# kcat/openal-soft

Measured on NVIDIA H100. Metric: voice-samples/s mixed (HRTF, bsinc24, 1024-frame updates), higher is better.
Workload: dtype f32

## Files before the change

### openal-soft_b200/csrc/b200mix.cu

```cuda
#include "../../include/b200mix.h"

#include <algorithm>
#include <cmath>
#include <cstdio>
#include <cstdlib>
#include <cstring>
#include <new>
#include <string>
#include <vector>

#include <cuda_runtime.h>

#include <dlfcn.h>

#include "mixer_kernels.cuh"
#include "effect_kernels.cuh"
#include "shard_kernels.cuh"
#include "panmix_tc.cuh"
#include "param_kernels.hpp"
#include "efx_kernels.hpp"
#include "resampler_tables.hpp"
#include "hrtf_store.hpp"
#include "adpcm.hpp"

using namespace b200mix;

namespace {

thread_local std::string g_create_error;

struct DevBuf {
    void *ptr{nullptr}; size_t bytes{0};
};

}

struct b200mix_device {
    b200mix_device_desc desc{};
    int cuda_dev{0};
    int num_sms{0};
    cudaStream_t stream{nullptr};
    std::string error;
    uint64_t launches{0};

    BsincTable bsinc[3];
    float *d_bsinc[3]{};
    float *d_cubic[2]{};

    VoiceRec *d_voices{nullptr};
    BufferRec *d_buffers{nullptr};
    std::vector<BufferRec> h_buffers;
    std::vector<uint32_t> h_vbuf;
    std::vector<uint32_t> h_bufrefs;
    float2 *d_hrtf_tgt{nullptr}, *d_hrtf_old{nullptr};
    float *d_dry_cur{nullptr}, *d_dry_tgt{nullptr}, *d_send_cur{nullptr}, *d_send_tgt{nullptr};
    VoiceResult *d_results{nullptr};
    b200mix_voice_result *h_results{nullptr};
    char *d_outblock{nullptr}, *h_outblock{nullptr}; size_t out_real_bytes{0};

    uint32_t dry_alloc_ch{0};
    float *d_dry{nullptr}, *d_real{nullptr}, *d_wet{nullptr};
    float *d_partial{nullptr}; size_t partial_floats{0};
    float *d_accum_sum{nullptr};
    float *d_carry[2]{};
    int carry_idx{0};
    float *h_real{nullptr};

    uint32_t dec_channels{0}, dec_ir{0};
    float2 *d_dec_coef{nullptr}; float *d_dec_hfscale{nullptr}, *d_dec_state{nullptr};
    float *d_temp{nullptr}, *d_temp2{nullptr};
    uint32_t amb_in{0}; bool amb_dual{false};
    float *d_amb_hf{nullptr}, *d_amb_lf{nullptr}, *d_amb_state{nullptr};
    bool dry_active{false};
    float *d_uhj_state{nullptr}, *d_uhj_scratch{nullptr};
    uint32_t stab_center{B200MIX_NO_SLOT};
    float stab_coeff{0.0f};
    float *d_stab_state{nullptr};
    uint32_t bs2b_level{0};
    float *d_bs2b{nullptr};
    uint32_t uhj_fir{0};
    float *d_uhj_fir_state{nullptr}, *d_uhj_fir_coef{nullptr};

    char *h_arena{nullptr}, *d_arena{nullptr};
    VoiceUpdate *h_upd{nullptr};
    uint32_t stage_cap{0};
    cudaEvent_t stage_done{nullptr};
    bool stage_busy{false};

    std::vector<SlotRec> h_slots;
    SlotRec *d_slots{nullptr};
    std::vector<std::vector<void*>> slot_allocs;
    uint32_t active_slots{0};
    float *d_xscratch{nullptr};
    uint32_t *d_sendinfo{nullptr};
    FilterRec *d_filt{nullptr};
    FilterUpdate *h_fupd{nullptr}, *d_fupd{nullptr};
    uint32_t fupd_cap{0};
    cudaEvent_t fstage_done{nullptr};
    bool fstage_busy{false};
    float *d_fscratch{nullptr};
    uint32_t fscratch_rows{0};
    float *d_dline{nullptr};
    std::vector<uint8_t> h_dfilt;
    std::vector<uint32_t> h_order2;
    uint32_t *d_order2{nullptr};
    uint32_t num_order2{0};
    bool order2_dirty{false};
    std::vector<uint32_t> h_send_slot;
    std::vector<uint32_t> h_slot_start;
    std::vector<SendEntry> h_entries;
    uint32_t *d_slot_start{nullptr};
    SendEntry *d_entries{nullptr};
    uint32_t num_entries{0};
    bool sends_dirty{true};
    struct EfxHost { bool used{false}; EfxParams p{}; EfxDev *dev{nullptr}; uint32_t mod_index{0}, mod_range{1};
        uint32_t lfo_offset{0}, lfo_range{1}; };
    std::vector<EfxHost> efx;
    EfxSlotView *d_efx_views{nullptr};
    uint32_t efx_slots{0};
    uint32_t pshift_slots{0};
    bool efx_ready{false};
    float2 *d_twiddle{nullptr};
    float *d_cubic_filter{nullptr};
    uint32_t reverb_slots{0};

    float2 *d_st_fields{nullptr}; uint2 *d_st_elevs{nullptr}; float2 *d_st_coeffs{nullptr};
    uint8_t *d_st_delays{nullptr}; uint32_t st_num_fields{0}, st_ir{0};
    uint4 *d_qhdr{nullptr}; uint32_t *d_queue{nullptr};
    LimiterDev *d_limiter{nullptr};
    float *d_limiter_delay{nullptr};
    uint32_t *d_dc_delay{nullptr}; float *d_dc_gain{nullptr}, *d_dc_buf{nullptr};
    void *d_outbuf{nullptr}, *h_outbuf{nullptr};
    struct RvHost {
        bool used{false};
        int cur{0}, state{4};
        uint32_t fade[2]{1u, 1u};
        uint32_t offset{0};
        ReverbDev h[2];
        ReverbDev *dev{nullptr};
    };
    std::vector<RvHost> rv;
    std::vector<uint32_t> h_target;
    uint32_t num_stages{1}; bool any_target{false};
    bool reverb_upmix{false};
    bool mid_render{false}; uint32_t mid_frames{0};
    bool real_overwrite{false};
    std::vector<uint8_t> h_hrtf;
    std::vector<SendEntry> h_dry_entries;
    SendEntry *d_dry_entries{nullptr};
    uint32_t *d_dry_slot_start{nullptr};
    uint32_t num_dry_entries{0};
    bool dry_entries_dirty{true};
    float *d_dry_partial{nullptr};
    float *d_dry_geff{nullptr};
    float *d_send_geff{nullptr};
    float4 *d_dry_gramp{nullptr}, *d_send_gramp{nullptr};
    float *d_send_partial{nullptr};
    uint32_t send_partial_chunks{0}, max_slot_entries{0};
    bool profile{false};
    cudaEvent_t ev_mix0{nullptr}, ev_mix1{nullptr};
    bool ev_valid{false};
    static constexpr int kStages = 8;
    cudaEvent_t ev_stage[kStages + 1]{};
    bool stage_valid{false}; int profile_level{0};

    std::vector<uint8_t> h_active;
    std::vector<uint32_t> h_cost;
    std::vector<uint32_t> h_order;
    uint32_t *d_order{nullptr};
    uint32_t num_order{0};
    bool order_dirty{true};

    char *h_src{nullptr}, *d_src{nullptr}; uint32_t src_cap{0};
    cudaEvent_t src_done{nullptr}; bool src_busy{false};
    bool dev_filters{false};
    bool panmix_tc{false};
    bool mix_gather_only{false};

    struct Shard {
        uint32_t rank{0}, world{1}; int transport{0};
        char *own{nullptr}; size_t bytes{0};
        char *peer[kShardMaxWorld]{};
        size_t off_real{0}, off_wet{0}, real_floats{0}, wet_src_floats{0};
        uint32_t owned_max{0};
        uint32_t epoch{0};
        uint32_t *d_counters{nullptr};
        uint32_t *h_status{nullptr};
        cudaEvent_t ev[4]{};
        bool ev_wet{false}, ev_real{false};
        void *nccl_lib{nullptr}; void *comm{nullptr};
        int (*reduce)(const void*, void*, size_t, int, int, int, void*, cudaStream_t){nullptr};
        int (*allreduce)(const void*, void*, size_t, int, int, void*, cudaStream_t){nullptr};
        int (*comm_destroy)(void*){nullptr};
    } shard;

    uint32_t ir_pad{0};
    uint32_t voice_hi{0};
    int mix_variant{0}; int mix_groups{2}; int mix_gs{64}; int mix_cdr{0};
    uint32_t reverb_seq{0};
    size_t mix_smem{0}; int mix_blocks_per_sm{1};
};

namespace {

#define CUDA_TRY(dev, expr) do { cudaError_t e_ = (expr); if(e_ != cudaSuccess) {            \
    (dev)->error = std::string(#expr) + ": " + cudaGetErrorString(e_); return B200MIX_ERR_CUDA; } } while(0)

template<typename T>
int dev_alloc(b200mix_device *d, T *&p, size_t count, bool zero = true)
{
    p = nullptr;
    if(count == 0) return B200MIX_OK;
    CUDA_TRY(d, cudaMalloc(reinterpret_cast<void**>(&p), count*sizeof(T)));
    if(zero) CUDA_TRY(d, cudaMemsetAsync(p, 0, count*sizeof(T), d->stream));
    return B200MIX_OK;
}

using MixKernel = void(*)(const MixParams);

struct Variant { MixKernel fn; int gs, groups, cdr; size_t smem; bool hrtf; };

template<int GS, int GROUPS, bool HRTF, int CDR, int OPT, int FP>
Variant make_variant()
{
    return Variant{k_mix_voices<GS, GROUPS, HRTF, CDR, OPT, FP>, GS, GROUPS, CDR,
        sizeof(GroupSmem<GS, OPT, FP>)*GROUPS, HRTF};
}

Variant get_variant(int idx)
{
    switch(idx)
    {
    case 0: return make_variant<64, 2, true, 0, 17, 64>();
    case 1: return make_variant<64, 2, true, 0, 19, 128>();
    case 2: return make_variant<64, 2, false, 4, 1, 8>();
    default: return make_variant<64, 2, false, 0, 1, 8>();
    }
}

constexpr uint32_t kDryChunksMax = 128;

int ensure_dry_park(b200mix_device *d)
{
    const b200mix_device_desc &dd = d->desc;
    if(d->d_dry_entries) return B200MIX_OK;
    if(!d->d_xscratch)
        if(int rc = dev_alloc(d, d->d_xscratch, size_t(dd.max_voices)*kLine)) return rc;
    if(!d->d_sendinfo)
        if(int rc = dev_alloc(d, d->d_sendinfo, dd.max_voices)) return rc;
    if(int rc = dev_alloc(d, d->d_dry_entries, dd.max_voices)) return rc;
    if(dd.dry_channels > 4u && dd.dry_channels <= uint32_t(kPmN))
    {
        CUDA_TRY(d, cudaFuncSetAttribute(k_panmix_tc, cudaFuncAttributeMaxDynamicSharedMemorySize,
            kPmStages*kPmStageBytes + 1024));
        const char *simt = std::getenv("B200MIX_PANMIX_SIMT");
        d->panmix_tc = !(simt && simt[0] == '1');
    }
    if(int rc = dev_alloc(d, d->d_dry_slot_start, 2)) return rc;
    if(int rc = dev_alloc(d, d->d_dry_partial, size_t(kDryChunksMax)*dd.dry_channels*kLine)) return rc;
    if(int rc = dev_alloc(d, d->d_dry_geff, size_t(dd.max_voices)*dd.dry_channels)) return rc;
    if(int rc = dev_alloc(d, d->d_dry_gramp, size_t(dd.max_voices)*dd.dry_channels)) return rc;
    return B200MIX_OK;
}

static size_t align16(size_t v) { return (v + 15u) & ~size_t(15); }

int ensure_stage(b200mix_device *d, uint32_t n)
{
    if(n <= d->stage_cap) return B200MIX_OK;
    const b200mix_device_desc &dd = d->desc;
    if(d->stage_cap)
    {
        cudaStreamSynchronize(d->stream);
        cudaFreeHost(d->h_arena); cudaFree(d->d_arena);
        d->h_arena = nullptr; d->d_arena = nullptr;
    }
    const uint32_t cap = std::max<uint32_t>(n, 256u);
    const size_t bytes = align16(size_t(cap)*sizeof(VoiceUpdate))
        + align16(size_t(cap)*std::max<size_t>(size_t(dd.ir_size)*2, 4)*sizeof(float))
        + align16(size_t(cap)*dd.dry_channels*sizeof(float))
        + align16(size_t(cap)*dd.num_sends*dd.wet_channels*sizeof(float)) + 64;
    CUDA_TRY(d, cudaMallocHost(reinterpret_cast<void**>(&d->h_arena), bytes));
    CUDA_TRY(d, cudaMalloc(reinterpret_cast<void**>(&d->d_arena), bytes));
    d->h_upd = reinterpret_cast<VoiceUpdate*>(d->h_arena);
    d->stage_cap = cap;
    return B200MIX_OK;
}

const BsincTable *bsinc_for(const b200mix_device *d, uint32_t resampler)
{
    if(resampler < B200MIX_RESAMPLER_FAST_BSINC12 || resampler > B200MIX_RESAMPLER_BSINC48)
        return nullptr;
    return &d->bsinc[(resampler - B200MIX_RESAMPLER_FAST_BSINC12) >> 1];
}

}

extern "C" {

static void shard_release(b200mix_device *d);
static int ensure_filters(b200mix_device *d);

uint32_t b200mix_version(void) { return (1u<<16) | 1u; }

const char *b200mix_last_error(const b200mix_device *dev)
{ return dev ? dev->error.c_str() : g_create_error.c_str(); }

int b200mix_create(const b200mix_device_desc *desc, b200mix_device **out)
{
    if(!desc || !out || desc->struct_size != sizeof(b200mix_device_desc))
    { g_create_error = "bad descriptor"; return B200MIX_ERR_INVALID; }
    if(desc->dry_channels > B200MIX_MAX_DRY_CHANNELS || desc->wet_channels > B200MIX_MAX_WET_CHANNELS
        || desc->num_sends > B200MIX_MAX_SENDS || desc->ir_size > B200MIX_HRIR_LENGTH
        || desc->real_channels > B200MIX_MAX_DRY_CHANNELS || desc->max_voices == 0)
    { g_create_error = "descriptor out of range"; return B200MIX_ERR_INVALID; }
    if((desc->post_process == B200MIX_POST_UHJ && desc->dry_channels < 3)
        || (desc->post_process == B200MIX_POST_TSME && desc->dry_channels < 4))
    { g_create_error = "UHJ post-process needs W,X,Y dry channels"; return B200MIX_ERR_INVALID; }
    if((desc->post_process == B200MIX_POST_HRTF || desc->post_process == B200MIX_POST_UHJ
        || desc->post_process == B200MIX_POST_TSME)
        && (desc->real_left >= desc->real_channels || desc->real_right >= desc->real_channels))
    { g_create_error = "real_left/real_right outside RealOut"; return B200MIX_ERR_INVALID; }

    auto *d = new(std::nothrow) b200mix_device{};
    if(!d) { g_create_error = "out of host memory"; return B200MIX_ERR_NOMEM; }
    d->desc = *desc;
    if(const char *g = std::getenv("B200MIX_MIX_GATHER")) d->mix_gather_only = g[0] == '1';
    auto fail = [&](int code) { g_create_error = d->error; b200mix_destroy(d); return code; };

    int count = 0;
    if(cudaGetDeviceCount(&count) != cudaSuccess || count < 1)
    { d->error = "no CUDA device: the b200mix mixer has no CPU path"; return fail(B200MIX_ERR_CUDA); }
    if(desc->cuda_device >= 0) d->cuda_dev = desc->cuda_device;
    else if(cudaGetDevice(&d->cuda_dev) != cudaSuccess) d->cuda_dev = 0;
    if(cudaSetDevice(d->cuda_dev) != cudaSuccess)
    { d->error = "cudaSetDevice failed"; return fail(B200MIX_ERR_CUDA); }
    cudaDeviceProp prop{};
    if(cudaGetDeviceProperties(&prop, d->cuda_dev) != cudaSuccess)
    { d->error = "cudaGetDeviceProperties failed"; return fail(B200MIX_ERR_CUDA); }
    d->num_sms = prop.multiProcessorCount;
    if(cudaStreamCreateWithFlags(&d->stream, cudaStreamNonBlocking) != cudaSuccess)
    { d->error = "cudaStreamCreate failed"; return fail(B200MIX_ERR_CUDA); }
    if(cudaEventCreateWithFlags(&d->stage_done, cudaEventDisableTiming) != cudaSuccess)
    { d->error = "cudaEventCreate failed"; return fail(B200MIX_ERR_CUDA); }

    auto run = [&]() -> int {
        d->bsinc[0] = BuildBsincTable(60, 11, 2);
        d->bsinc[1] = BuildBsincTable(60, 23, 2);
        d->bsinc[2] = BuildBsincTable(80, 47, 1);
        for(int i = 0;i < 3;++i)
        {
            if(int rc = dev_alloc(d, d->d_bsinc[i], d->bsinc[i].tab.size(), false)) return rc;
            CUDA_TRY(d, cudaMemcpyAsync(d->d_bsinc[i], d->bsinc[i].tab.data(),
                d->bsinc[i].tab.size()*sizeof(float), cudaMemcpyHostToDevice, d->stream));
        }
        const std::vector<float> cubic[2] = {BuildSplineTable(), BuildGaussianTable()};
        for(int i = 0;i < 2;++i)
        {
            if(int rc = dev_alloc(d, d->d_cubic[i], cubic[i].size(), false)) return rc;
            CUDA_TRY(d, cudaMemcpyAsync(d->d_cubic[i], cubic[i].data(), cubic[i].size()*sizeof(float),
                cudaMemcpyHostToDevice, d->stream));
        }
        CUDA_TRY(d, cudaStreamSynchronize(d->stream));

        const b200mix_device_desc &dd = d->desc;
        d->ir_pad = (dd.ir_size + 7u) & ~7u;
        if(int rc = dev_alloc(d, d->d_voices, dd.max_voices)) return rc;
        if(int rc = dev_alloc(d, d->d_buffers, std::max(dd.max_buffers, 1u))) return rc;
        d->h_buffers.assign(std::max(dd.max_buffers, 1u), BufferRec{});
        d->h_vbuf.assign(dd.max_voices, B200MIX_NO_SLOT);
        d->h_bufrefs.assign(std::max(dd.max_buffers, 1u), 0u);
        if(dd.ir_size)
        {
            if(int rc = dev_alloc(d, d->d_hrtf_tgt, size_t(dd.max_voices)*d->ir_pad)) return rc;
            if(int rc = dev_alloc(d, d->d_hrtf_old, size_t(dd.max_voices)*d->ir_pad)) return rc;
        }
        if(int rc = dev_alloc(d, d->d_dry_cur, size_t(dd.max_voices)*std::max(dd.dry_channels, 1u))) return rc;
        if(int rc = dev_alloc(d, d->d_dry_tgt, size_t(dd.max_voices)*std::max(dd.dry_channels, 1u))) return rc;
        if(dd.num_sends && dd.wet_channels)
        {
            const size_t per = size_t(dd.num_sends)*dd.wet_channels;
            if(int rc = dev_alloc(d, d->d_send_cur, dd.max_voices*per)) return rc;
            if(int rc = dev_alloc(d, d->d_send_tgt, dd.max_voices*per)) return rc;
        }
        if(int rc = dev_alloc(d, d->d_order, dd.max_voices)) return rc;
        d->h_active.assign(dd.max_voices, 0);
        d->h_cost.assign(dd.max_voices, 0);
        d->h_hrtf.assign(dd.max_voices, 0);

        const bool hrtfDev = dd.ir_size > 0;
        d->mix_variant = hrtfDev ? (dd.ir_size <= 64 ? 0 : 1) : (dd.dry_channels <= 4 ? 2 : 3);
        const Variant var = get_variant(d->mix_variant);
        d->mix_gs = var.gs; d->mix_groups = var.groups; d->mix_cdr = var.cdr; d->mix_smem = var.smem;
        CUDA_TRY(d, cudaFuncSetAttribute(var.fn, cudaFuncAttributeMaxDynamicSharedMemorySize, int(var.smem)));
        int perSm = 0;
        CUDA_TRY(d, cudaOccupancyMaxActiveBlocksPerMultiprocessor(&perSm, var.fn, var.gs*var.groups, var.smem));
        d->mix_blocks_per_sm = std::max(perSm, 1);

        d->dry_alloc_ch = std::max<uint32_t>(std::max(dd.dry_channels, 1u), uint32_t(var.cdr));
        if(int rc = dev_alloc(d, d->d_dry, size_t(d->dry_alloc_ch)*kLine)) return rc;
        {
            const size_t realFloats = size_t(std::max(dd.real_channels, 1u))*kLine;
            static_assert(sizeof(VoiceResult) == 16 && sizeof(b200mix_voice_result) == 16, "result layout");
            const size_t blockBytes = realFloats*sizeof(float) + size_t(dd.max_voices)*sizeof(VoiceResult);
            char *blk = nullptr;
            if(int rc = dev_alloc(d, blk, blockBytes)) return rc;
            d->d_outblock = blk;
            d->d_results = reinterpret_cast<VoiceResult*>(blk + realFloats*sizeof(float));
            CUDA_TRY(d, cudaMallocHost(reinterpret_cast<void**>(&d->h_outblock), blockBytes));
            d->h_real = reinterpret_cast<float*>(d->h_outblock);
            d->h_results = reinterpret_cast<b200mix_voice_result*>(d->h_outblock + realFloats*sizeof(float));
            d->out_real_bytes = realFloats*sizeof(float);
            if(dd.post_process == B200MIX_POST_NONE) d->d_real = d->d_dry;
            else d->d_real = reinterpret_cast<float*>(blk);
        }
        if(dd.max_slots && dd.wet_channels)
            if(int rc = dev_alloc(d, d->d_wet, size_t(dd.max_slots)*dd.wet_channels*kLine)) return rc;
        const size_t maxRows = size_t(d->num_sms)*d->mix_blocks_per_sm;
        d->partial_floats = maxRows*(hrtfDev ? 2*kAccumLen : 0) + maxRows*size_t(var.cdr)*kLine;
        if(int rc = dev_alloc(d, d->d_partial, std::max<size_t>(2*d->partial_floats, 4))) return rc;
        if(int rc = dev_alloc(d, d->d_accum_sum, 2*kAccumLen)) return rc;
        if(int rc = dev_alloc(d, d->d_carry[0], 2*kHrirLen)) return rc;
        if(int rc = dev_alloc(d, d->d_carry[1], 2*kHrirLen)) return rc;
        if(int rc = dev_alloc(d, d->d_temp, size_t(std::max(dd.dry_channels, 1u))*kLine)) return rc;
        if(int rc = dev_alloc(d, d->d_temp2, size_t(std::max(dd.dry_channels, 1u))*kLine)) return rc;
        if(dd.max_slots && dd.wet_channels && dd.num_sends)
        {
            d->h_slots.assign(dd.max_slots, SlotRec{});
            d->slot_allocs.assign(dd.max_slots, {});
            if(int rc = dev_alloc(d, d->d_slots, dd.max_slots)) return rc;
            if(int rc = dev_alloc(d, d->d_xscratch, size_t(dd.max_voices)*kLine)) return rc;
            if(int rc = dev_alloc(d, d->d_sendinfo, dd.max_voices)) return rc;
            if(int rc = dev_alloc(d, d->d_send_geff, size_t(dd.max_voices)*dd.num_sends*dd.wet_channels)) return rc;
            if(int rc = dev_alloc(d, d->d_send_gramp, size_t(dd.max_voices)*dd.num_sends*dd.wet_channels)) return rc;
            d->h_send_slot.assign(size_t(dd.max_voices)*B200MIX_MAX_SENDS, B200MIX_NO_SLOT);
            if(int rc = dev_alloc(d, d->d_slot_start, dd.max_slots + 1)) return rc;
            if(int rc = dev_alloc(d, d->d_entries, size_t(dd.max_voices)*dd.num_sends)) return rc;
            std::vector<float2> tw(128);
            for(int k = 0;k < 128;++k)
            {
                const double a = -2.0*3.14159265358979323846*double(k)/256.0;
                tw[k] = make_float2(float(std::cos(a)), float(std::sin(a)));
            }
            const std::vector<float> cf = BuildCubicFilter();
            if(int rc = dev_alloc(d, d->d_cubic_filter, cf.size(), false)) return rc;
            CUDA_TRY(d, cudaMemcpyAsync(d->d_cubic_filter, cf.data(), cf.size()*sizeof(float),
                cudaMemcpyHostToDevice, d->stream));
            CUDA_TRY(d, cudaStreamSynchronize(d->stream));
            if(int rc = dev_alloc(d, d->d_twiddle, 128, false)) return rc;
            CUDA_TRY(d, cudaMemcpyAsync(d->d_twiddle, tw.data(), 128*sizeof(float2),
                cudaMemcpyHostToDevice, d->stream));
            CUDA_TRY(d, cudaStreamSynchronize(d->stream));
        }
        if(dd.post_process == B200MIX_POST_UHJ || dd.post_process == B200MIX_POST_TSME)
        {
            if(int rc = dev_alloc(d, d->d_uhj_state, 64)) return rc;
            if(int rc = dev_alloc(d, d->d_uhj_scratch, 5*1025)) return rc;
        }
        if(int rc = ensure_stage(d, std::min(dd.max_voices, 4096u))) return rc;
        CUDA_TRY(d, cudaStreamSynchronize(d->stream));
        return B200MIX_OK;
    };
    int rc;
    try { rc = run(); }
    catch(const std::exception &e) { d->error = e.what(); rc = B200MIX_ERR_NOMEM; }
    if(rc != B200MIX_OK) return fail(rc);
    *out = d;
    return B200MIX_OK;
}

void b200mix_destroy(b200mix_device *d)
{
    if(!d) return;
    if(d->stream) cudaStreamSynchronize(d->stream);
    shard_release(d);
    for(auto &b : d->h_buffers) if(b.data) cudaFree(const_cast<void*>(b.data));
    for(int i = 0;i < 3;++i) cudaFree(d->d_bsinc[i]);
    for(int i = 0;i < 2;++i) cudaFree(d->d_cubic[i]);
    cudaFree(d->d_voices); cudaFree(d->d_buffers); cudaFree(d->d_hrtf_tgt); cudaFree(d->d_hrtf_old);
    cudaFree(d->d_dry_cur); cudaFree(d->d_dry_tgt); cudaFree(d->d_send_cur); cudaFree(d->d_send_tgt);
    cudaFree(d->d_outblock); cudaFreeHost(d->h_outblock); cudaFree(d->d_order);
    cudaFree(d->d_dry); cudaFree(d->d_wet); cudaFree(d->d_partial); cudaFree(d->d_accum_sum);
    cudaFree(d->d_carry[0]); cudaFree(d->d_carry[1]);
    cudaFree(d->d_dec_coef); cudaFree(d->d_dec_hfscale); cudaFree(d->d_dec_state);
    cudaFree(d->d_temp); cudaFree(d->d_temp2);
    cudaFree(d->d_amb_hf); cudaFree(d->d_amb_lf); cudaFree(d->d_amb_state);
    cudaFree(d->d_uhj_state); cudaFree(d->d_uhj_scratch);
    cudaFree(d->d_uhj_fir_state); cudaFree(d->d_uhj_fir_coef); cudaFree(d->d_bs2b); cudaFree(d->d_stab_state);
    for(auto &v : d->slot_allocs) for(void *p : v) cudaFree(p);
    cudaFree(d->d_slots); cudaFree(d->d_xscratch); cudaFree(d->d_sendinfo);
    cudaFree(d->d_filt); cudaFree(d->d_fupd); cudaFree(d->d_fscratch);
    cudaFree(d->d_dline); cudaFree(d->d_order2); cudaFree(d->d_qhdr); cudaFree(d->d_queue);
    cudaFree(d->d_outbuf); if(d->h_outbuf) cudaFreeHost(d->h_outbuf);
    cudaFree(d->d_limiter); cudaFree(d->d_limiter_delay);
    cudaFree(d->d_dc_delay); cudaFree(d->d_dc_gain); cudaFree(d->d_dc_buf);
    cudaFree(d->d_st_fields); cudaFree(d->d_st_elevs); cudaFree(d->d_st_coeffs); cudaFree(d->d_st_delays);
    cudaFree(d->d_dry_entries); cudaFree(d->d_dry_slot_start); cudaFree(d->d_dry_partial);
    cudaFree(d->d_dry_geff); cudaFree(d->d_send_geff); cudaFree(d->d_send_partial);
    cudaFree(d->d_dry_gramp); cudaFree(d->d_send_gramp);
    if(d->h_fupd) cudaFreeHost(d->h_fupd);
    if(d->fstage_done) cudaEventDestroy(d->fstage_done);
    cudaFree(d->d_slot_start); cudaFree(d->d_entries); cudaFree(d->d_twiddle); cudaFree(d->d_cubic_filter);
    cudaFree(d->d_efx_views);
    cudaFreeHost(d->h_arena); cudaFree(d->d_arena);
    if(d->h_src) cudaFreeHost(d->h_src);
    cudaFree(d->d_src);
    if(d->src_done) cudaEventDestroy(d->src_done);
    if(d->stage_done) cudaEventDestroy(d->stage_done);
    if(d->ev_mix0) cudaEventDestroy(d->ev_mix0);
    if(d->ev_mix1) cudaEventDestroy(d->ev_mix1);
    for(cudaEvent_t e : d->ev_stage) if(e) cudaEventDestroy(e);
    if(d->stream) cudaStreamDestroy(d->stream);
    delete d;
}

int b200mix_set_hrtf_decoder(b200mix_device *d, uint32_t channels, uint32_t ir_size,
    const float *coeffs, const float *hf_scale, const float *splitter_coeff)
{
    if(!d || channels != d->desc.dry_channels || ir_size > B200MIX_HRIR_LENGTH || !coeffs
        || !hf_scale || !splitter_coeff || d->desc.post_process != B200MIX_POST_HRTF)
    { if(d) d->error = "set_hrtf_decoder: bad arguments"; return B200MIX_ERR_INVALID; }
    CUDA_TRY(d, cudaSetDevice(d->cuda_dev));
    cudaFree(d->d_dec_coef); cudaFree(d->d_dec_hfscale); cudaFree(d->d_dec_state);
    d->dec_channels = channels; d->dec_ir = ir_size;
    if(int rc = dev_alloc(d, d->d_dec_coef, size_t(channels)*ir_size, false)) return rc;
    if(int rc = dev_alloc(d, d->d_dec_hfscale, channels, false)) return rc;
    if(int rc = dev_alloc(d, d->d_dec_state, size_t(channels)*4)) return rc;
    std::vector<float> st(size_t(channels)*4, 0.0f);
    for(uint32_t c = 0;c < channels;++c) st[c*4] = splitter_coeff[c];
    CUDA_TRY(d, cudaMemcpyAsync(d->d_dec_coef, coeffs, size_t(channels)*ir_size*2*sizeof(float),
        cudaMemcpyHostToDevice, d->stream));
    CUDA_TRY(d, cudaMemcpyAsync(d->d_dec_hfscale, hf_scale, channels*sizeof(float),
        cudaMemcpyHostToDevice, d->stream));
    CUDA_TRY(d, cudaMemcpyAsync(d->d_dec_state, st.data(), st.size()*sizeof(float),
        cudaMemcpyHostToDevice, d->stream));
    CUDA_TRY(d, cudaStreamSynchronize(d->stream));
    return B200MIX_OK;
}

int b200mix_set_ambi_decoder(b200mix_device *d, uint32_t in_channels, const float *gains_hf,
    const float *gains_lf, float xover_coeff)
{
    if(!d || in_channels != d->desc.dry_channels || !gains_hf
        || d->desc.post_process != B200MIX_POST_AMBIDEC)
    { if(d) d->error = "set_ambi_decoder: bad arguments"; return B200MIX_ERR_INVALID; }
    CUDA_TRY(d, cudaSetDevice(d->cuda_dev));
    cudaFree(d->d_amb_hf); cudaFree(d->d_amb_lf); cudaFree(d->d_amb_state);
    d->d_amb_lf = nullptr;
    const size_t n = size_t(in_channels)*d->desc.real_channels;
    d->amb_in = in_channels; d->amb_dual = gains_lf != nullptr;
    if(int rc = dev_alloc(d, d->d_amb_hf, n, false)) return rc;
    CUDA_TRY(d, cudaMemcpyAsync(d->d_amb_hf, gains_hf, n*sizeof(float), cudaMemcpyHostToDevice, d->stream));
    if(gains_lf)
    {
        if(int rc = dev_alloc(d, d->d_amb_lf, n, false)) return rc;
        CUDA_TRY(d, cudaMemcpyAsync(d->d_amb_lf, gains_lf, n*sizeof(float), cudaMemcpyHostToDevice, d->stream));
    }
    std::vector<float> st(size_t(in_channels)*4, 0.0f);
    for(uint32_t c = 0;c < in_channels;++c) st[c*4] = xover_coeff;
    if(int rc = dev_alloc(d, d->d_amb_state, st.size(), false)) return rc;
    CUDA_TRY(d, cudaMemcpyAsync(d->d_amb_state, st.data(), st.size()*sizeof(float),
        cudaMemcpyHostToDevice, d->stream));
    CUDA_TRY(d, cudaStreamSynchronize(d->stream));
    return B200MIX_OK;
}

int b200mix_buffer_data(b200mix_device *d, uint32_t buffer, uint32_t sample_type, uint32_t channels,
    uint32_t frames, const void *data, size_t bytes)
{
    if(!d) return B200MIX_ERR_INVALID;
    static const size_t sz[] = {1, 2, 4, 4, 8, 1, 1};
    if(buffer >= d->desc.max_buffers || sample_type > B200MIX_FMT_ALAW || channels < 1 || !data)
    { d->error = "buffer_data: bad arguments"; return B200MIX_ERR_INVALID; }
    const size_t need = size_t(frames)*channels*sz[sample_type];
    if(bytes < need) { d->error = "buffer_data: short data"; return B200MIX_ERR_INVALID; }
    CUDA_TRY(d, cudaSetDevice(d->cuda_dev));
    BufferRec &h = d->h_buffers[buffer];
    if(h.data && d->h_bufrefs[buffer])
    { d->error = "buffer_data: the buffer is attached to an active voice (AL_INVALID_OPERATION)"; return B200MIX_ERR_INVALID; }
    if(h.data)
    {
        CUDA_TRY(d, cudaStreamSynchronize(d->stream));
        cudaFree(const_cast<void*>(h.data));
        h = BufferRec{};
    }
    void *p = nullptr;
    CUDA_TRY(d, cudaMalloc(&p, need + 16));
    CUDA_TRY(d, cudaMemcpyAsync(p, data, need, cudaMemcpyHostToDevice, d->stream));
    h.data = p; h.frames = frames; h.type = sample_type; h.channels = channels;
    CUDA_TRY(d, cudaMemcpyAsync(d->d_buffers + buffer, &h, sizeof(BufferRec), cudaMemcpyHostToDevice,
        d->stream));
    return B200MIX_OK;
}

int b200mix_buffer_data_adpcm(b200mix_device *d, uint32_t buffer, uint32_t sample_type,
    uint32_t channels, uint32_t samples_per_block, uint32_t blocks, const void *data, size_t bytes)
{
    if(!d) return B200MIX_ERR_INVALID;
    const bool ms = sample_type == B200MIX_FMT_MSADPCM;
    if((sample_type != B200MIX_FMT_IMA4 && !ms) || channels < 1 || channels > 2 || !data
        || !AdpcmBlockValid(ms, samples_per_block))
    { d->error = "buffer_data_adpcm: bad arguments"; return B200MIX_ERR_INVALID; }
    if(bytes < AdpcmBlockBytes(ms, channels, samples_per_block)*blocks
        || uint64_t(blocks)*samples_per_block > 0x7fffffffull)
    { d->error = "buffer_data_adpcm: short data"; return B200MIX_ERR_INVALID; }
    std::vector<int16_t> pcm(size_t(blocks)*samples_per_block*channels);
    if(ms) DecodeMSADPCM(static_cast<const uint8_t*>(data), channels, samples_per_block, blocks, pcm.data());
    else DecodeIMA4(static_cast<const uint8_t*>(data), channels, samples_per_block, blocks, pcm.data());
    const int rc = b200mix_buffer_data(d, buffer, B200MIX_FMT_I16, channels, blocks*samples_per_block,
        pcm.data(), pcm.size()*sizeof(int16_t));
    if(rc == B200MIX_OK) CUDA_TRY(d, cudaStreamSynchronize(d->stream));
    return rc;
}

int b200mix_buffer_free(b200mix_device *d, uint32_t buffer)
{
    if(!d || buffer >= d->desc.max_buffers) return B200MIX_ERR_INVALID;
    CUDA_TRY(d, cudaSetDevice(d->cuda_dev));
    BufferRec &h = d->h_buffers[buffer];
    if(h.data && d->h_bufrefs[buffer])
    { d->error = "buffer_free: the buffer is attached to an active voice; stop the voice first"; return B200MIX_ERR_INVALID; }
    if(h.data)
    {
        CUDA_TRY(d, cudaStreamSynchronize(d->stream));
        cudaFree(const_cast<void*>(h.data));
        h = BufferRec{};
        CUDA_TRY(d, cudaMemcpyAsync(d->d_buffers + buffer, &h, sizeof(BufferRec),
            cudaMemcpyHostToDevice, d->stream));
    }
    return B200MIX_OK;
}

static int update_stages(b200mix_device *d)
{
    const uint32_t ns = uint32_t(d->h_slots.size());
    if(d->h_target.size() != ns) d->h_target.assign(ns, B200MIX_NO_SLOT);
    std::vector<uint32_t> depth(ns, 0);
    uint32_t maxd = 0; d->any_target = false;
    for(uint32_t sl = 0;sl < ns;++sl)
    {
        uint32_t hops = 0;
        for(uint32_t t = d->h_target[sl];t != B200MIX_NO_SLOT && hops <= ns;t = d->h_target[t]) ++hops;
        depth[sl] = hops;
        if(d->h_slots[sl].type) { maxd = std::max(maxd, hops); if(hops) d->any_target = true; }
    }
    d->num_stages = maxd + 1u;
    for(uint32_t sl = 0;sl < ns;++sl)
    {
        d->h_slots[sl].stage = d->h_slots[sl].type ? maxd - std::min(depth[sl], maxd) : 0u;
        d->h_slots[sl].target = d->h_target[sl];
    }
    if(ns && d->d_slots)
    {
        CUDA_TRY(d, cudaMemcpyAsync(d->d_slots, d->h_slots.data(), ns*sizeof(SlotRec), cudaMemcpyHostToDevice, d->stream));
        CUDA_TRY(d, cudaStreamSynchronize(d->stream));
    }
    if(ns && d->d_efx_views)
    {
        std::vector<EfxSlotView> views(ns, EfxSlotView{nullptr, nullptr, 0u, 0u});
        for(uint32_t sl = 0;sl < ns;++sl)
            if(d->h_slots[sl].type >= B200MIX_EFFECT_ECHO && sl < d->efx.size() && d->efx[sl].used)
                views[sl] = EfxSlotView{d->efx[sl].dev, d->h_slots[sl].lines, d->h_slots[sl].stage, 0u};
        CUDA_TRY(d, cudaMemcpyAsync(d->d_efx_views, views.data(), ns*sizeof(EfxSlotView), cudaMemcpyHostToDevice, d->stream));
        CUDA_TRY(d, cudaStreamSynchronize(d->stream));
    }
    return B200MIX_OK;
}

static void free_slot(b200mix_device *d, uint32_t slot)
{
    cudaStreamSynchronize(d->stream);
    for(void *p : d->slot_allocs[slot]) cudaFree(p);
    d->slot_allocs[slot].clear();
    if(d->h_slots[slot].type) --d->active_slots;
    if(d->h_slots[slot].type == B200MIX_EFFECT_REVERB) --d->reverb_slots;
    if(d->h_slots[slot].type >= B200MIX_EFFECT_ECHO)
    {
        --d->efx_slots;
        if(d->h_slots[slot].type == B200MIX_EFFECT_PSHIFTER) --d->pshift_slots;
        if(slot < d->efx.size()) d->efx[slot] = b200mix_device::EfxHost{};
    }
    if(slot < d->rv.size()) d->rv[slot].used = false;
    d->h_slots[slot] = SlotRec{};
    if(d->d_slots)
    {
        cudaMemcpyAsync(d->d_slots + slot, &d->h_slots[slot], sizeof(SlotRec), cudaMemcpyHostToDevice, d->stream);
        cudaStreamSynchronize(d->stream);
    }
}

int b200mix_slot_disable(b200mix_device *d, uint32_t slot)
{
    if(!d || slot >= d->h_slots.size()) { if(d) d->error = "slot_disable: bad slot"; return B200MIX_ERR_INVALID; }
    CUDA_TRY(d, cudaSetDevice(d->cuda_dev));
    free_slot(d, slot);
    return update_stages(d);
}

int b200mix_slot_convolution(b200mix_device *d, uint32_t slot, uint32_t ir_channels,
    uint32_t ir_frames, const float *ir)
{
    if(!d || slot >= d->h_slots.size() || !ir_channels || ir_channels > 16 || !ir_frames || !ir)
    { if(d) d->error = "slot_convolution: bad arguments (or the device has no sends/slots)"; return B200MIX_ERR_INVALID; }
    CUDA_TRY(d, cudaSetDevice(d->cuda_dev));
    free_slot(d, slot);
    CUDA_TRY(d, cudaFuncSetAttribute(k_conv_mac, cudaFuncAttributeMaxDynamicSharedMemorySize, int(sizeof(ConvMacSmem))));
    SlotRec r{};
    r.type = B200MIX_EFFECT_CONVOLUTION; r.channels = ir_channels; r.frames = ir_frames;
    const uint32_t nseg = std::max<uint32_t>((ir_frames + kConvBlock - 1)/kConvBlock, 2u) - 1u;
    r.segs = nseg;
    auto alloc = [&](auto *&p, size_t count) -> int {
        if(int rc = dev_alloc(d, p, count)) return rc;
        d->slot_allocs[slot].push_back(p);
        return B200MIX_OK;
    };
    if(int rc = alloc(r.H, size_t(ir_channels)*nseg*kConvFft)) return rc;
    if(int rc = alloc(r.X, size_t(nseg + kConvMaxBlocks)*kConvFft)) return rc;
    if(int rc = alloc(r.head, size_t(ir_channels)*kConvBlock)) return rc;
    if(int rc = alloc(r.inbuf, kConvFft)) return rc;
    if(int rc = alloc(r.ov, size_t(ir_channels)*kConvFft)) return rc;
    if(int rc = alloc(r.yspec, size_t(ir_channels)*kConvMaxChunks*kConvMaxBlocks*kConvFft)) return rc;
    if(int rc = alloc(r.lines, size_t(ir_channels)*kLine)) return rc;
    if(int rc = alloc(r.gains, size_t(2)*ir_channels*32)) return rc;
    if(int rc = alloc(r.gtgt, size_t(ir_channels)*32)) return rc;

    std::vector<float> H(size_t(ir_channels)*nseg*kConvFft, 0.0f), head(size_t(ir_channels)*kConvBlock, 0.0f);
    std::vector<double> cs(kConvFft), sn(kConvFft);
    for(int k = 0;k < kConvFft;++k)
    {
        cs[k] = std::cos(2.0*3.14159265358979323846*k/kConvFft);
        sn[k] = std::sin(2.0*3.14159265358979323846*k/kConvFft);
    }
    for(uint32_t c = 0;c < ir_channels;++c)
    {
        const float *h = ir + size_t(c)*ir_frames;
        for(uint32_t k = 0;k < uint32_t(kConvBlock) && k < ir_frames;++k) head[c*kConvBlock + k] = h[k];
        for(uint32_t sg = 0;sg < nseg;++sg)
        {
            const size_t base = size_t(kConvBlock)*(sg + 1);
            float *dst = H.data() + (size_t(c)*nseg + sg)*kConvFft;
            const uint32_t cnt = base < ir_frames ? std::min<uint32_t>(kConvBlock, uint32_t(ir_frames - base)) : 0u;
            for(int bin = 0;bin <= kConvBlock;++bin)
            {
                double re = 0.0, im = 0.0;
                for(uint32_t j = 0;j < cnt;++j)
                {
                    const int ph = int((uint64_t(bin)*j) % kConvFft);
                    re += double(h[base + j])*cs[ph];
                    im -= double(h[base + j])*sn[ph];
                }
                const double sc = 1.0/double(kConvFft);
                if(bin == 0) dst[0] = float(re*sc);
                else if(bin == kConvBlock) dst[1] = float(re*sc);
                else { dst[bin*2] = float(re*sc); dst[bin*2+1] = float(im*sc); }
            }
        }
    }
    CUDA_TRY(d, cudaMemcpyAsync(r.H, H.data(), H.size()*sizeof(float), cudaMemcpyHostToDevice, d->stream));
    CUDA_TRY(d, cudaMemcpyAsync(r.head, head.data(), head.size()*sizeof(float), cudaMemcpyHostToDevice, d->stream));
    d->h_slots[slot] = r;
    CUDA_TRY(d, cudaMemcpyAsync(d->d_slots + slot, &d->h_slots[slot], sizeof(SlotRec), cudaMemcpyHostToDevice, d->stream));
    CUDA_TRY(d, cudaStreamSynchronize(d->stream));
    ++d->active_slots;
    d->dry_active = true;
    return update_stages(d);
}

static void reverb_fill_params(ReverbDev &h, const b200mix_reverb_params *p)
{
    std::memcpy(h.early_tap, p->early_tap, sizeof(h.early_tap)); h.early_tap_coeff = p->early_tap_coeff;
    std::memcpy(h.late_tap, p->late_tap, sizeof(h.late_tap));
    h.mix_x = p->mix_x; h.mix_y = p->mix_y;
    std::memcpy(h.filter_lp, p->filter_lp, sizeof(h.filter_lp));
    std::memcpy(h.filter_hp, p->filter_hp, sizeof(h.filter_hp));
    h.early_ap_coeff = p->early_ap_coeff;
    std::memcpy(h.early_ap_offset, p->early_ap_offset, sizeof(h.early_ap_offset));
    std::memcpy(h.early_offset, p->early_offset, sizeof(h.early_offset));
    h.early_coeff = p->early_coeff;
    std::memcpy(h.late_offset, p->late_offset, sizeof(h.late_offset));
    h.density_gain = p->density_gain;
    std::memcpy(h.t60_mid_gain, p->t60_mid_gain, sizeof(h.t60_mid_gain));
    std::memcpy(h.t60_hf, p->t60_hf, sizeof(h.t60_hf)); std::memcpy(h.t60_lf, p->t60_lf, sizeof(h.t60_lf));
    h.mod_step = p->mod_step; h.mod_depth = p->mod_depth; h.late_ap_coeff = p->late_ap_coeff;
    std::memcpy(h.late_ap_offset, p->late_ap_offset, sizeof(h.late_ap_offset));
    h.upmix = p->upmix ? 1u : 0u; h.order_scale[0] = p->order_scale[0]; h.order_scale[1] = p->order_scale[1];
    h.split_coeff = p->splitter_coeff;
}

static int reverb_check_params(b200mix_device *d, const b200mix_reverb_params *p)
{
    auto pow2 = [](uint32_t v) { return v >= 4u && !(v & (v-1u)); };
    if(!pow2(p->main_len) || !pow2(p->late_in_len) || !pow2(p->early_ap_len) || !pow2(p->early_len)
        || !pow2(p->late_ap_len) || !pow2(p->late_len) || !p->late_offset[0] || !p->late_ap_offset[0])
// ... 551 lines not shown
                if(int rc = ensure_dry_park(d)) return rc;
        }
        const uint8_t hv = hrtfMode ? 1 : 0;
        if(d->h_hrtf[p.voice] != hv) { d->h_hrtf[p.voice] = hv; d->dry_entries_dirty = true; }
        const uint8_t act = stopped ? 0 : 1;
        uint32_t cost = p.resampler >= 2u ? 4u : 2u;
        if(const BsincTable *t = bsinc_for(d, p.resampler)) cost = t->m[0];
        if(d->h_active[p.voice] != act || (!d->h_cost[p.voice] && act)) { d->order_dirty = true; d->h_cost[p.voice] = cost; }
        d->h_active[p.voice] = act;
        d->voice_hi = std::max(d->voice_hi, p.voice + 1u);
        const uint32_t nb = (!stopped && (p.flags & B200MIX_VF_STATIC)) ? p.buffer : B200MIX_NO_SLOT;
        uint32_t &ob = d->h_vbuf[p.voice];
        if(ob != nb)
        {
            if(ob != B200MIX_NO_SLOT) --d->h_bufrefs[ob];
            if(nb != B200MIX_NO_SLOT) ++d->h_bufrefs[nb];
            ob = nb;
        }
    }

    const uint32_t paths = 1u + dd.num_sends;
    const size_t inBytes = align16(size_t(n)*sizeof(b200mix_source_voice)) + align16(size_t(n)*sizeof(b200mix_source_props));
    if(d->src_busy) { CUDA_TRY(d, cudaEventSynchronize(d->src_done)); d->src_busy = false; }
    if(n > d->src_cap)
    {
        CUDA_TRY(d, cudaStreamSynchronize(d->stream));
        if(d->h_src) cudaFreeHost(d->h_src);
        cudaFree(d->d_src); d->h_src = nullptr; d->d_src = nullptr;
        const uint32_t cap = std::max(n, 2u*d->src_cap);
        const size_t in = align16(size_t(cap)*sizeof(b200mix_source_voice)) + align16(size_t(cap)*sizeof(b200mix_source_props));
        const size_t out = align16(size_t(cap)*sizeof(VoiceUpdate)) + align16(size_t(cap)*16)
            + align16(size_t(cap)*std::max(dd.dry_channels, 1u)*4) + align16(size_t(cap)*std::max(dd.num_sends*dd.wet_channels, 1u)*4)
            + align16(size_t(cap)*(1u + B200MIX_MAX_SENDS)*8) + align16(size_t(cap)*paths*sizeof(FilterUpdate));
        CUDA_TRY(d, cudaMallocHost(reinterpret_cast<void**>(&d->h_src), in));
        CUDA_TRY(d, cudaMalloc(reinterpret_cast<void**>(&d->d_src), in + out + 64));
        if(!d->src_done) CUDA_TRY(d, cudaEventCreateWithFlags(&d->src_done, cudaEventDisableTiming));
        d->src_cap = cap;
    }
    std::memcpy(d->h_src, voices, size_t(n)*sizeof(b200mix_source_voice));
    const size_t offProps = align16(size_t(n)*sizeof(b200mix_source_voice));
    std::memcpy(d->h_src + offProps, props, size_t(n)*sizeof(b200mix_source_props));
    CUDA_TRY(d, cudaMemcpyAsync(d->d_src, d->h_src, inBytes, cudaMemcpyHostToDevice, d->stream));
    CUDA_TRY(d, cudaEventRecord(d->src_done, d->stream));
    d->src_busy = true;

    CalcVoicesParams Q{};
    Q.voices = reinterpret_cast<const b200mix_source_voice*>(d->d_src);
    Q.props = reinterpret_cast<const b200mix_source_props*>(d->d_src + offProps);
    Q.n = n; Q.listener = *listener;
    Q.device_rate = env->device_rate; Q.num_sends = dd.num_sends; Q.render_mode = env->render_mode;
    Q.cd = dd.dry_channels; Q.cw = dd.wet_channels; Q.ir = dd.ir_size;
    if(!hrtfMode)
    {
        Q.dry_channels = env->dry.channels;
        for(uint32_t c = 0;c < env->dry.channels;++c) { Q.dry_scale[c] = env->dry.scale[c]; Q.dry_index[c] = env->dry.index[c]; }
    }
    for(uint32_t s = 0;s < dd.num_sends;++s)
    {
        Q.wet_channels[s] = env->wet[s].channels;
        for(uint32_t c = 0;c < env->wet[s].channels;++c) { Q.wet_scale[s][c] = env->wet[s].scale[c]; Q.wet_index[s][c] = env->wet[s].index[c]; }
    }
    for(int t = 0;t < 3;++t)
    {
        Q.bsinc[t].scaleBase = d->bsinc[t].scaleBase; Q.bsinc[t].scaleRange = d->bsinc[t].scaleRange;
        for(unsigned k = 0;k < kBsincScales;++k) { Q.bsinc[t].m[k] = d->bsinc[t].m[k]; Q.bsinc[t].filterOffset[k] = d->bsinc[t].filterOffset[k]; }
    }
    size_t off = inBytes;
    auto carve = [&](size_t bytes) { char *p = d->d_src + off; off += align16(bytes); return p; };
    Q.updates = reinterpret_cast<VoiceUpdate*>(carve(size_t(n)*sizeof(VoiceUpdate)));
    Q.dirs = reinterpret_cast<float4*>(carve(size_t(n)*16));
    Q.dry = reinterpret_cast<float*>(carve(size_t(n)*std::max(dd.dry_channels, 1u)*4));
    Q.send = (dd.num_sends && dd.wet_channels)
        ? reinterpret_cast<float*>(carve(size_t(n)*dd.num_sends*dd.wet_channels*4)) : nullptr;
    Q.gains_hflf = reinterpret_cast<float*>(carve(size_t(n)*(1u + B200MIX_MAX_SENDS)*8));
    Q.fupd = reinterpret_cast<FilterUpdate*>(carve(size_t(n)*paths*sizeof(FilterUpdate)));
    const bool filters = d->d_filt != nullptr;
    CUDA_TRY(d, launch_calc_voices(Q, filters, d->stream));
    d->launches += filters ? 2 : 1;

    ApplyParams A{};
    A.voices = d->d_voices; A.updates = Q.updates;
    if(hrtfMode)
    {
        A.dirs = Q.dirs;
        A.st_fields = d->d_st_fields; A.st_elevs = d->d_st_elevs; A.st_coeffs = d->d_st_coeffs;
        A.st_delays = d->d_st_delays; A.st_num_fields = d->st_num_fields; A.st_ir = d->st_ir;
    }
    else A.dry = Q.dry;
    A.send = Q.send;
    A.hrtf_tgt = d->d_hrtf_tgt; A.hrtf_old = d->d_hrtf_old;
    A.dry_cur = d->d_dry_cur; A.dry_tgt = d->d_dry_tgt;
    A.send_cur = d->d_send_cur; A.send_tgt = d->d_send_tgt;
    A.ir = dd.ir_size; A.ir_pad = d->ir_pad; A.cd = dd.dry_channels; A.cw = dd.wet_channels;
    A.num_sends = dd.num_sends;
    A.filt = d->d_filt; A.filt_paths = paths;
    A.qhdr = d->d_qhdr;
    k_apply_updates<<<n, 64, 0, d->stream>>>(A);
    ++d->launches;
    if(filters)
    {
        k_apply_filter_updates<<<(2u*n*paths + 127u)/128u, 128, 0, d->stream>>>(d->d_filt, paths, Q.fupd, n*paths);
        ++d->launches;
    }
    CUDA_TRY(d, cudaGetLastError());
    return B200MIX_OK;
}

int b200mix_get_voice_targets(b200mix_device *d, uint32_t voice, uint32_t *step, float bsinc[4],
    float *hrtf_gain, uint32_t hrtf_delay[2], float *hrtf_coeffs, float *dry_gains, float *send_gains,
    float *filters)
{
    if(!d || voice >= d->desc.max_voices) return B200MIX_ERR_INVALID;
    const b200mix_device_desc &dd = d->desc;
    CUDA_TRY(d, cudaSetDevice(d->cuda_dev));
    CUDA_TRY(d, cudaStreamSynchronize(d->stream));
    VoiceRec rec;
    CUDA_TRY(d, cudaMemcpy(&rec, d->d_voices + voice, offsetof(VoiceRec, prev), cudaMemcpyDeviceToHost));
    if(step) *step = rec.step;
    if(bsinc)
    {
        bsinc[0] = rec.bsinc_sf;
        std::memcpy(&bsinc[1], &rec.bsinc_m, 4); std::memcpy(&bsinc[2], &rec.bsinc_l, 4);
        std::memcpy(&bsinc[3], &rec.bsinc_off, 4);
    }
    if(hrtf_gain) *hrtf_gain = rec.tgt_gain;
    if(hrtf_delay) { hrtf_delay[0] = rec.tgt_delay0; hrtf_delay[1] = rec.tgt_delay1; }
    if(hrtf_coeffs && d->d_hrtf_tgt)
        CUDA_TRY(d, cudaMemcpy(hrtf_coeffs, d->d_hrtf_tgt + size_t(voice)*d->ir_pad, size_t(dd.ir_size)*8, cudaMemcpyDeviceToHost));
    if(dry_gains && dd.dry_channels)
        CUDA_TRY(d, cudaMemcpy(dry_gains, d->d_dry_tgt + size_t(voice)*dd.dry_channels, size_t(dd.dry_channels)*4, cudaMemcpyDeviceToHost));
    if(send_gains && d->d_send_tgt)
        CUDA_TRY(d, cudaMemcpy(send_gains, d->d_send_tgt + size_t(voice)*dd.num_sends*dd.wet_channels,
            size_t(dd.num_sends)*dd.wet_channels*4, cudaMemcpyDeviceToHost));
    if(filters)
    {
        const uint32_t paths = 1u + dd.num_sends;
        for(uint32_t pth = 0;pth < paths;++pth)
        {
            float *o = filters + size_t(pth)*11;
            for(int k = 0;k < 11;++k) o[k] = k == 1 ? 1.0f : (k == 6 ? 1.0f : 0.0f);
            if(!d->d_filt) continue;
            FilterRec fr;
            CUDA_TRY(d, cudaMemcpy(&fr, d->d_filt + size_t(voice)*paths + pth, sizeof(fr), cudaMemcpyDeviceToHost));
            o[0] = fr.active ? 1.0f : 0.0f;
            for(int k = 0;k < 5;++k) { o[1+k] = fr.tgt[0][k]; o[6+k] = fr.tgt[1][k]; }
        }
    }
    return B200MIX_OK;
}

int b200mix_voice_queue(b200mix_device *d, uint32_t voice, uint32_t count, const uint32_t *buffers,
    uint32_t loop_index)
{
    if(!d) return B200MIX_ERR_INVALID;
    const b200mix_device_desc &dd = d->desc;
    if(voice >= dd.max_voices || (count && !buffers))
    { d->error = "voice_queue: bad arguments"; return B200MIX_ERR_INVALID; }
    if(count > B200MIX_MAX_QUEUE)
    { d->error = "voice_queue: more than B200MIX_MAX_QUEUE items"; return B200MIX_ERR_UNSUPPORTED; }
    if(loop_index != B200MIX_NO_LOOP && loop_index >= count)
    { d->error = "voice_queue: loop index outside the list"; return B200MIX_ERR_INVALID; }
    QueueSet Q{};
    Q.voice = voice; Q.count = count; Q.loop = loop_index;
    for(uint32_t i = 0;i < count;++i)
    {
        if(buffers[i] >= dd.max_buffers || !d->h_buffers[buffers[i]].data)
        { d->error = "voice_queue: buffer id without data"; return B200MIX_ERR_INVALID; }
        Q.items[i] = buffers[i];
    }
    CUDA_TRY(d, cudaSetDevice(d->cuda_dev));
    if(!d->d_qhdr)
    {
        if(int rc = dev_alloc(d, d->d_qhdr, dd.max_voices)) return rc;
        if(int rc = dev_alloc(d, d->d_queue, size_t(dd.max_voices)*kMaxQueue)) return rc;
    }
    k_set_queue<<<1, 32, 0, d->stream>>>(d->d_voices, d->d_qhdr, d->d_queue, Q);
    ++d->launches;
    CUDA_TRY(d, cudaGetLastError());
    return B200MIX_OK;
}

static int ensure_filters(b200mix_device *d)
{
    if(d->d_filt) return B200MIX_OK;
    const b200mix_device_desc &dd = d->desc;
    const uint32_t paths = 1u + dd.num_sends;
    const size_t count = size_t(dd.max_voices)*paths;
    if(int rc = dev_alloc(d, d->d_filt, count, false)) return rc;
    k_filter_init<<<unsigned((count*32u + 255u)/256u), 256, 0, d->stream>>>(d->d_filt, count);
    ++d->launches;
    CUDA_TRY(d, cudaGetLastError());
    CUDA_TRY(d, cudaEventCreateWithFlags(&d->fstage_done, cudaEventDisableTiming));
    if(!d->d_xscratch)
        if(int rc = dev_alloc(d, d->d_xscratch, size_t(dd.max_voices)*kLine)) return rc;
    if(!d->d_sendinfo)
        if(int rc = dev_alloc(d, d->d_sendinfo, dd.max_voices)) return rc;
    if(int rc = dev_alloc(d, d->d_dline, size_t(dd.max_voices)*kLine)) return rc;
    if(int rc = dev_alloc(d, d->d_order2, dd.max_voices)) return rc;
    d->h_dfilt.assign(dd.max_voices, 0);
    return B200MIX_OK;
}

int b200mix_voices_filters(b200mix_device *d, uint32_t n, const b200mix_voice_filter *filters)
{
    static_assert(sizeof(FilterUpdate) == sizeof(b200mix_voice_filter), "FilterUpdate mirrors the ABI struct");
    if(!d) return B200MIX_ERR_INVALID;
    if(n == 0) return B200MIX_OK;
    if(!filters) { d->error = "voices_filters: null filters"; return B200MIX_ERR_INVALID; }
    const b200mix_device_desc &dd = d->desc;
    const uint32_t paths = 1u + dd.num_sends;
    for(uint32_t i = 0;i < n;++i)
        if(filters[i].voice >= dd.max_voices || filters[i].path >= paths)
        { d->error = "voices_filters: voice/path out of range"; return B200MIX_ERR_INVALID; }
    CUDA_TRY(d, cudaSetDevice(d->cuda_dev));
    if(int rc = ensure_filters(d)) return rc;
    for(uint32_t i = 0;i < n;++i)
        if(filters[i].path == 0)
        {
            const uint8_t act = filters[i].active ? 1 : 0;
            if(d->h_dfilt[filters[i].voice] != act) { d->h_dfilt[filters[i].voice] = act; d->order2_dirty = true; }
        }
    if(d->fstage_busy)
    {
        CUDA_TRY(d, cudaEventSynchronize(d->fstage_done));
        d->fstage_busy = false;
    }
    if(n > d->fupd_cap)
    {
        CUDA_TRY(d, cudaStreamSynchronize(d->stream));
        if(d->h_fupd) cudaFreeHost(d->h_fupd);
        cudaFree(d->d_fupd);
        d->h_fupd = nullptr; d->d_fupd = nullptr;
        const uint32_t cap = std::max(n, 2u*d->fupd_cap);
        CUDA_TRY(d, cudaMallocHost(reinterpret_cast<void**>(&d->h_fupd), size_t(cap)*sizeof(FilterUpdate)));
        CUDA_TRY(d, cudaMalloc(reinterpret_cast<void**>(&d->d_fupd), size_t(cap)*sizeof(FilterUpdate)));
        d->fupd_cap = cap;
    }
    std::memcpy(d->h_fupd, filters, size_t(n)*sizeof(FilterUpdate));
    CUDA_TRY(d, cudaMemcpyAsync(d->d_fupd, d->h_fupd, size_t(n)*sizeof(FilterUpdate),
        cudaMemcpyHostToDevice, d->stream));
    k_apply_filter_updates<<<(2u*n + 127u)/128u, 128, 0, d->stream>>>(d->d_filt, paths, d->d_fupd, n);
    ++d->launches;
    CUDA_TRY(d, cudaGetLastError());
    CUDA_TRY(d, cudaEventRecord(d->fstage_done, d->stream));
    d->fstage_busy = true;
    return B200MIX_OK;
}

static inline void stage_mark(b200mix_device *d, int i)
{ if(d->profile_level >= 2) cudaEventRecord(d->ev_stage[i], d->stream); }

static int render_phase_a(b200mix_device *d, uint32_t frames, bool want_results, bool force_sends)
{
    const b200mix_device_desc &dd = d->desc;
    if(frames < 1 || frames > B200MIX_LINE_SIZE)
    { d->error = "render: frames out of range"; return B200MIX_ERR_INVALID; }
    if(dd.post_process == B200MIX_POST_HRTF && !d->dec_channels)
    { d->error = "render: HRTF decoder not set"; return B200MIX_ERR_INVALID; }
    if(dd.post_process == B200MIX_POST_AMBIDEC && !d->amb_in)
    { d->error = "render: ambisonic decoder not set"; return B200MIX_ERR_INVALID; }
    CUDA_TRY(d, cudaSetDevice(d->cuda_dev));

    stage_mark(d, 0);
    if(d->dry_active || dd.post_process != B200MIX_POST_HRTF)
        CUDA_TRY(d, cudaMemsetAsync(d->d_dry, 0, size_t(d->dry_alloc_ch)*kLine*sizeof(float), d->stream));
    d->real_overwrite = dd.post_process == B200MIX_POST_HRTF && dd.real_channels == 2
        && dd.real_left != dd.real_right;
    if(d->d_real != d->d_dry && !d->real_overwrite)
        CUDA_TRY(d, cudaMemsetAsync(d->d_real, 0, size_t(dd.real_channels)*kLine*sizeof(float), d->stream));
    if(d->d_wet)
        CUDA_TRY(d, cudaMemsetAsync(d->d_wet, 0, size_t(dd.max_slots)*dd.wet_channels*kLine*sizeof(float), d->stream));

    if(d->order_dirty)
    {
        d->h_order.clear();
        for(uint32_t v = 0;v < d->voice_hi;++v) if(d->h_active[v]) d->h_order.push_back(v);
        std::stable_sort(d->h_order.begin(), d->h_order.end(),
            [d](uint32_t a, uint32_t b) { return d->h_cost[a] > d->h_cost[b]; });
        d->num_order = uint32_t(d->h_order.size());
        if(d->num_order)
        {
            CUDA_TRY(d, cudaMemcpyAsync(d->d_order, d->h_order.data(), d->num_order*sizeof(uint32_t),
                cudaMemcpyHostToDevice, d->stream));
            CUDA_TRY(d, cudaStreamSynchronize(d->stream));
        }
        d->order_dirty = false;
        d->order2_dirty = true;
        d->dry_entries_dirty = true;
    }
    if(d->d_filt && d->order2_dirty)
    {
        d->h_order2.clear();
        for(uint32_t v : d->h_order) if(d->dev_filters || d->h_dfilt[v]) d->h_order2.push_back(v);
        d->num_order2 = uint32_t(d->h_order2.size());
        if(d->num_order2)
        {
            CUDA_TRY(d, cudaMemcpyAsync(d->d_order2, d->h_order2.data(), d->num_order2*sizeof(uint32_t),
                cudaMemcpyHostToDevice, d->stream));
            CUDA_TRY(d, cudaStreamSynchronize(d->stream));
        }
        d->order2_dirty = false;
    }
    const Variant var = get_variant(d->mix_variant);
    const uint32_t nv = std::max(d->voice_hi, 1u);
    const uint32_t maxBlocks = uint32_t(d->num_sms*d->mix_blocks_per_sm);
    const uint32_t blocks = std::max(1u, std::min(maxBlocks, (d->num_order + var.groups - 1)/var.groups));
    const size_t rows = size_t(blocks);

    MixParams P{};
    P.voices = d->d_voices; P.buffers = d->d_buffers;
    P.hrtf_tgt = d->d_hrtf_tgt; P.hrtf_old = d->d_hrtf_old;
    P.dry_cur = d->d_dry_cur; P.dry_tgt = d->d_dry_tgt;
    P.send_cur = d->d_send_cur; P.send_tgt = d->d_send_tgt;
    P.dry = d->d_dry; P.wet = d->d_wet; P.partial = d->d_partial;
    P.results = want_results ? d->d_results : nullptr;
    for(int i = 0;i < 3;++i) P.bsinc_tab[i] = d->d_bsinc[i];
    for(int i = 0;i < 2;++i) P.cubic_tab[i] = d->d_cubic[i];
    P.max_voices = nv; P.frames = frames; P.ir = dd.ir_size; P.ir_pad = d->ir_pad;
    P.cd = dd.dry_channels; P.cw = dd.wet_channels; P.num_sends = dd.num_sends;
    P.max_buffers = dd.max_buffers;
    P.order = d->d_order; P.num_order = d->num_order;
    P.xscratch = d->d_xscratch; P.sendinfo = d->d_sendinfo;
    P.filt = d->d_filt; P.filt_paths = 1u + dd.num_sends;
    P.qhdr = d->d_qhdr; P.queue = d->d_queue;
    P.gather_only = d->mix_gather_only ? 1u : 0u;
    stage_mark(d, 1);
    if(d->profile) cudaEventRecord(d->ev_mix0, d->stream);
    var.fn<<<blocks, var.gs*var.groups, var.smem, d->stream>>>(P);
    if(d->profile) { cudaEventRecord(d->ev_mix1, d->stream); d->ev_valid = true; }
    ++d->launches;
    CUDA_TRY(d, cudaGetLastError());

    stage_mark(d, 2);
    size_t rows2 = 0;
    if(d->d_filt && d->num_order2)
    {
        FilterRunParams FP{};
        FP.filt = d->d_filt; FP.filt_paths = 1u + dd.num_sends; FP.sendinfo = d->d_sendinfo;
        FP.direct_order = d->d_order2; FP.num_direct = d->num_order2;
        FP.xscratch = d->d_xscratch; FP.dline = d->d_dline; FP.frames = frames;
        k_filters<<<(d->num_order2 + 31u)/32u, 32, 0, d->stream>>>(FP);
        ++d->launches;
        const uint32_t blocks2 = std::max(1u, std::min(maxBlocks, (d->num_order2 + var.groups - 1)/var.groups));
        rows2 = blocks2;
        MixParams P2 = P;
        P2.pass = 1u; P2.dline = d->d_dline;
        P2.order = d->d_order2; P2.num_order = d->num_order2;
        P2.partial = d->d_partial + d->partial_floats;
        P2.results = nullptr;
        var.fn<<<blocks2, var.gs*var.groups, var.smem, d->stream>>>(P2);
        ++d->launches;
        CUDA_TRY(d, cudaGetLastError());
    }

    stage_mark(d, 3);
    if(var.hrtf)
    {
        const uint32_t len = 2*kAccumLen;
        k_reduce_rows<<<(len/4 + kReduceCols - 1)/kReduceCols, 1024, 0, d->stream>>>(d->d_partial, uint32_t(rows), len,
            d->d_accum_sum, 0);
        ++d->launches;
        if(rows2)
        {
            k_reduce_rows<<<(len/4 + kReduceCols - 1)/kReduceCols, 1024, 0, d->stream>>>(d->d_partial + d->partial_floats,
                uint32_t(rows2), len, d->d_accum_sum, 1);
            ++d->launches;
        }
    }
    if(var.cdr > 0)
    {
        const uint32_t len = uint32_t(var.cdr)*kLine;
        const float *pd = d->d_partial + (var.hrtf ? rows*(2*kAccumLen) : 0);
        k_reduce_rows<<<(len/4 + kReduceCols - 1)/kReduceCols, 1024, 0, d->stream>>>(pd, uint32_t(rows), len, d->d_dry, 1);
        ++d->launches;
        if(rows2)
        {
            const float *pd2 = d->d_partial + d->partial_floats + (var.hrtf ? rows2*(2*kAccumLen) : 0);
            k_reduce_rows<<<(len/4 + kReduceCols - 1)/kReduceCols, 1024, 0, d->stream>>>(pd2, uint32_t(rows2), len, d->d_dry, 1);
            ++d->launches;
        }
    }
    CUDA_TRY(d, cudaGetLastError());

    stage_mark(d, 4);
    if(var.cdr == 0 && d->d_dry_entries)
    {
        if(d->dry_entries_dirty)
        {
            d->h_dry_entries.clear();
            for(uint32_t v = 0;v < d->voice_hi;++v)
                if(d->h_active[v] && !d->h_hrtf[v]) d->h_dry_entries.push_back(SendEntry{v, 0u});
            d->num_dry_entries = uint32_t(d->h_dry_entries.size());
            const uint32_t ss[2] = {0u, d->num_dry_entries};
            CUDA_TRY(d, cudaMemcpyAsync(d->d_dry_slot_start, ss, sizeof(ss), cudaMemcpyHostToDevice, d->stream));
            if(d->num_dry_entries)
                CUDA_TRY(d, cudaMemcpyAsync(d->d_dry_entries, d->h_dry_entries.data(),
                    d->num_dry_entries*sizeof(SendEntry), cudaMemcpyHostToDevice, d->stream));
            CUDA_TRY(d, cudaStreamSynchronize(d->stream));
            d->dry_entries_dirty = false;
        }
        if(d->num_dry_entries)
        {
            SendMixParams DM{};
            DM.slot_start = d->d_dry_slot_start; DM.entries = d->d_dry_entries; DM.sendinfo = d->d_sendinfo;
            DM.xscratch = d->d_xscratch; DM.send_cur = d->d_dry_cur; DM.send_tgt = d->d_dry_tgt;
            DM.wet = d->d_dry; DM.frames = frames; DM.cw = dd.dry_channels; DM.num_sends = 1;
            DM.valid_bit = kSiDry; DM.dline = d->d_dline ? d->d_dline : d->d_xscratch;
            const uint32_t chunks = std::max(1u, std::min(kDryChunksMax, (d->num_dry_entries + 63u)/64u));
            DM.chunks = chunks; DM.partial = d->d_dry_partial; DM.geff = d->d_dry_geff; DM.gramp = d->d_dry_gramp;
            {
                const uint32_t tot = d->num_dry_entries*dd.dry_channels;
                k_send_gains_prepare<<<(tot + 127)/128, 128, 0, d->stream>>>(DM, d->num_dry_entries);
                ++d->launches;
            }
            const bool tc = d->panmix_tc && dd.dry_channels > 4u && dd.dry_channels <= uint32_t(kPmN)
                && frames == uint32_t(kLine) && chunks > 1u;
            const uint32_t tiles = tc ? 1u : (chunks > 1u ? uint32_t(kLine/128) : (frames + 127u)/128u);
            if(dd.dry_channels > 4u) k_send_mix<16><<<dim3(1, tiles, chunks), 256, 0, d->stream>>>(DM);
            else k_send_mix<4><<<dim3(1, tiles, chunks), 256, 0, d->stream>>>(DM);
            ++d->launches;
            if(tc)
            {
                PanMixTcParams TQ{d->d_dry_slot_start, d->d_dry_entries, d->d_sendinfo, d->d_xscratch,
                    d->d_dline, d->d_dry_geff, dd.dry_channels, chunks, d->d_dry_partial};
                k_panmix_tc<<<chunks, 128, kPmStages*kPmStageBytes + 1024, d->stream>>>(TQ);
                ++d->launches;
            }
            if(chunks > 1u)
            {
                const uint32_t len = dd.dry_channels*kLine;
                if(chunks <= 16u)
                    k_reduce_few<<<(len/4 + 255)/256, 256, 0, d->stream>>>(d->d_dry_partial, chunks, len, d->d_dry, 1);
                else
                k_reduce_rows<<<(len/4 + kReduceCols - 1)/kReduceCols, 1024, 0, d->stream>>>(
                    d->d_dry_partial, chunks, len, d->d_dry, 1);
                ++d->launches;
            }
            const uint32_t tot = d->num_dry_entries*dd.dry_channels;
            k_send_gains_update<<<(tot + 127)/128, 128, 0, d->stream>>>(DM, d->num_dry_entries);
            ++d->launches;
            CUDA_TRY(d, cudaGetLastError());
        }
    }

    stage_mark(d, 5);
    if((d->active_slots || force_sends) && d->d_wet && d->d_slot_start)
    {
        if(d->sends_dirty)
        {
            d->h_slot_start.assign(dd.max_slots + 1, 0);
            d->h_entries.clear();
            for(uint32_t sl = 0;sl < dd.max_slots;++sl)
            {
                d->h_slot_start[sl] = uint32_t(d->h_entries.size());
                for(uint32_t v = 0;v < d->voice_hi;++v)
                    for(uint32_t s2 = 0;s2 < dd.num_sends;++s2)
                        if(d->h_send_slot[size_t(v)*B200MIX_MAX_SENDS + s2] == sl)
                            d->h_entries.push_back(SendEntry{v, s2});
            }
            d->h_slot_start[dd.max_slots] = uint32_t(d->h_entries.size());
            d->num_entries = uint32_t(d->h_entries.size());
            d->max_slot_entries = 0;
            for(uint32_t sl = 0;sl < dd.max_slots;++sl)
                d->max_slot_entries = std::max(d->max_slot_entries, d->h_slot_start[sl+1] - d->h_slot_start[sl]);
            CUDA_TRY(d, cudaMemcpyAsync(d->d_slot_start, d->h_slot_start.data(),
                (dd.max_slots + 1)*sizeof(uint32_t), cudaMemcpyHostToDevice, d->stream));
            if(d->num_entries)
                CUDA_TRY(d, cudaMemcpyAsync(d->d_entries, d->h_entries.data(),
                    d->num_entries*sizeof(SendEntry), cudaMemcpyHostToDevice, d->stream));
            CUDA_TRY(d, cudaStreamSynchronize(d->stream));
            d->sends_dirty = false;
        }
        SendMixParams SM{};
        SM.slot_start = d->d_slot_start; SM.entries = d->d_entries; SM.sendinfo = d->d_sendinfo;
        SM.xscratch = d->d_xscratch; SM.send_cur = d->d_send_cur; SM.send_tgt = d->d_send_tgt;
        SM.wet = d->d_wet; SM.frames = frames; SM.cw = dd.wet_channels; SM.num_sends = dd.num_sends;
        SM.valid_bit = kSiSend; SM.chunks = 1;
        if(d->d_filt && d->num_entries)
        {
            if(d->fscratch_rows < d->num_entries)
            {
                CUDA_TRY(d, cudaStreamSynchronize(d->stream));
                cudaFree(d->d_fscratch); d->d_fscratch = nullptr; d->fscratch_rows = 0;
                const uint32_t rows = std::max(d->num_entries, 64u);
                CUDA_TRY(d, cudaMalloc(reinterpret_cast<void**>(&d->d_fscratch), size_t(rows)*kLine*sizeof(float)));
                CUDA_TRY(d, cudaMemsetAsync(d->d_fscratch, 0, size_t(rows)*kLine*sizeof(float), d->stream));
                d->fscratch_rows = rows;
            }
            SM.filt = d->d_filt; SM.filt_paths = 1u + dd.num_sends; SM.fscratch = d->d_fscratch;
            FilterRunParams FP{};
            FP.filt = d->d_filt; FP.filt_paths = 1u + dd.num_sends; FP.sendinfo = d->d_sendinfo;
            FP.entries = d->d_entries; FP.num_entries = d->num_entries;
            FP.xscratch = d->d_xscratch; FP.fscratch = d->d_fscratch; FP.frames = frames;
            k_filters<<<(d->num_entries + 31u)/32u, 32, 0, d->stream>>>(FP);
            ++d->launches;
        }
        SM.geff = d->d_send_geff; SM.gramp = d->d_send_gramp;
        if(d->num_entries)
        {
            const uint32_t tot = d->num_entries*dd.wet_channels;
            k_send_gains_prepare<<<(tot + 127)/128, 128, 0, d->stream>>>(SM, d->num_entries);
            ++d->launches;
        }
        {
            const uint32_t chunks = std::max(1u, std::min(16u, (d->max_slot_entries + 127u)/128u));
            if(chunks > 1u && d->send_partial_chunks < chunks)
            {
                CUDA_TRY(d, cudaStreamSynchronize(d->stream));
                cudaFree(d->d_send_partial); d->d_send_partial = nullptr; d->send_partial_chunks = 0;
                CUDA_TRY(d, cudaMalloc(reinterpret_cast<void**>(&d->d_send_partial),
                    size_t(chunks)*dd.max_slots*dd.wet_channels*kLine*sizeof(float)));
                d->send_partial_chunks = chunks;
            }
            SM.chunks = chunks; SM.partial = d->d_send_partial;
            const uint32_t tiles = chunks > 1u ? uint32_t(kLine/128) : (frames + 127u)/128u;
            if(dd.wet_channels > 4u) k_send_mix<16><<<dim3(dd.max_slots, tiles, chunks), 256, 0, d->stream>>>(SM);
            else k_send_mix<4><<<dim3(dd.max_slots, tiles, chunks), 256, 0, d->stream>>>(SM);
            ++d->launches;
            if(chunks > 1u)
            {
                const uint32_t len = dd.max_slots*dd.wet_channels*kLine;
                if(chunks <= 16u)
                    k_reduce_few<<<(len/4 + 255)/256, 256, 0, d->stream>>>(d->d_send_partial, chunks, len, d->d_wet, 1);
                else
                k_reduce_rows<<<(len/4 + kReduceCols - 1)/kReduceCols, 1024, 0, d->stream>>>(
                    d->d_send_partial, chunks, len, d->d_wet, 1);
                ++d->launches;
            }
        }
        if(d->num_entries)
        {
            const uint32_t tot = d->num_entries*dd.wet_channels;
            k_send_gains_update<<<(tot + 127)/128, 128, 0, d->stream>>>(SM, d->num_entries);
            ++d->launches;
        }
        CUDA_TRY(d, cudaGetLastError());
    }
    return B200MIX_OK;
}

static int render_phase_b(b200mix_device *d, uint32_t frames)
{
    const b200mix_device_desc &dd = d->desc;
    stage_mark(d, 6);
    if(d->active_slots)
    {
        ConvParams CP{};
        CP.slots = d->d_slots; CP.wet = d->d_wet; CP.twiddle = d->d_twiddle;
        CP.frames = frames; CP.cw = dd.wet_channels; CP.num_slots = dd.max_slots;
        uint32_t convCh = 1, convWork = 0, convSegs = 0;
        for(const SlotRec &sr : d->h_slots)
            if(sr.type == B200MIX_EFFECT_CONVOLUTION)
            { convCh = std::max(convCh, sr.channels); convWork += sr.channels; convSegs = std::max(convSegs, sr.segs); }
        CP.chunks = 1u;
        if(convWork)
            CP.chunks = std::max(1u, std::min(std::min(uint32_t(kConvMaxChunks), (convSegs + 17u)/18u),
                (4u*uint32_t(d->num_sms) + convWork - 1u)/convWork));
        if(d->reverb_slots)
        {
            for(uint32_t sl = 0;sl < d->rv.size();++sl)
            {
                b200mix_device::RvHost &R = d->rv[sl];
                if(!R.used || d->h_slots[sl].type != B200MIX_EFFECT_REVERB) continue;
                uint32_t mask = 1u << R.cur;
                if(R.state < 2) R.state = 2;
                if(R.state != 4)
                {
                    const int old = R.cur ^ 1;
                    if(R.state == 3)
                    {
                        if(int rc = reverb_clear_pipeline(d, sl, old)) return rc;
                        R.state = 4;
                    }
                    else
                    {
                        if(frames >= R.fade[old])
                        {
                            CUDA_TRY(d, cudaMemsetAsync(d->h_slots[sl].gtgt + size_t(old)*8*32, 0,
                                size_t(8)*32*sizeof(float), d->stream));
                            R.fade[old] = 0; R.state = 3;
                        }
                        else R.fade[old] -= frames;
                        mask |= 1u << old;
                    }
                }
                R.offset += frames;
                if(d->h_slots[sl].rv_mask != mask || d->h_slots[sl].rv_cur != uint32_t(R.cur))
                {
                    d->h_slots[sl].rv_mask = mask; d->h_slots[sl].rv_cur = uint32_t(R.cur);
                    CUDA_TRY(d, cudaMemcpyAsync(d->d_slots + sl, &d->h_slots[sl], sizeof(SlotRec),
                        cudaMemcpyHostToDevice, d->stream));
                    CUDA_TRY(d, cudaStreamSynchronize(d->stream));
                }
            }
        }
        SlotMixParams SP{};
        SP.slots = d->d_slots; SP.dry = d->d_dry; SP.frames = frames; SP.cd = dd.dry_channels;
        SP.num_slots = dd.max_slots; SP.wet = d->d_wet; SP.cw = dd.wet_channels;
        for(uint32_t st = 0;st < d->num_stages;++st)
        {
            if(d->reverb_slots)
            {
                ReverbParamsK RP{};
                RP.slots = d->d_slots; RP.wet = d->d_wet; RP.cubic = d->d_cubic_filter;
                RP.frames = frames; RP.cw = dd.wet_channels; RP.stage = st;
                RP.seq = ++d->reverb_seq;
                k_reverb_process<<<dim3(dd.max_slots, 2, 2), 128, 0, d->stream>>>(RP);
                k_reverb_commit<<<dd.max_slots, 2, 0, d->stream>>>(RP);
                d->launches += 2;
                if(d->reverb_upmix)
                {
                    k_reverb_upmix<<<dim3(dd.max_slots, 2), 256, 8*kLine*sizeof(float), d->stream>>>(RP);
                    ++d->launches;
                }
            }
            CP.stage = st; SP.stage = st;
            if(d->efx_slots)
            {
                EfxRunParams EQ{d->d_efx_views, d->d_wet, frames, dd.wet_channels, st, d->d_cubic_filter};
                CUDA_TRY(d, launch_efx_process(EQ, dd.max_slots, d->stream));
                ++d->launches;
                if(d->pshift_slots)
                {
                    CUDA_TRY(d, launch_efx_pshift(EQ, dd.max_slots, d->stream));
                    ++d->launches;
                }
            }
            if(convWork)
            {
                k_conv_input<<<dd.max_slots, 128, 0, d->stream>>>(CP);
                k_conv_mac<<<dim3(dd.max_slots, convCh, CP.chunks), 128, sizeof(ConvMacSmem), d->stream>>>(CP);
                k_conv_ifft<<<dim3(dd.max_slots, convCh, kConvMaxBlocks), 128, 0, d->stream>>>(CP);
                k_conv_output<<<dim3(dd.max_slots, convCh), 128, 0, d->stream>>>(CP);
                d->launches += 4;
            }
            k_slot_output_mix<<<dim3((frames + 127)/128, dd.dry_channels), 128, 0, d->stream>>>(SP);
            ++d->launches;
            if(d->any_target)
            {
                k_slot_target_mix<<<dim3((frames + 127)/128, dd.max_slots), 128, 0, d->stream>>>(SP);
                ++d->launches;
            }
        }
        k_slot_gains_commit<<<dd.max_slots, 64, 0, d->stream>>>(SP);
        ++d->launches;
        for(auto &eh : d->efx)
        {
            if(eh.used && eh.p.type == B200MIX_EFFECT_MODULATOR) eh.mod_index = (eh.mod_index + frames) % eh.mod_range;
            if(eh.used && eh.p.type == B200MIX_EFFECT_CHORUS) eh.lfo_offset = (eh.lfo_offset + frames) % eh.lfo_range;
        }
        CUDA_TRY(d, cudaGetLastError());
    }

    stage_mark(d, 7);
    switch(dd.post_process)
    {
    case B200MIX_POST_HRTF:
    {
        PostHrtfParams Q{};
        Q.accum_sum = d->d_accum_sum; Q.carry_in = d->d_carry[d->carry_idx];
        Q.carry_out = d->d_carry[d->carry_idx^1];
        Q.dry = d->d_dry; Q.real = d->d_real; Q.dec_coef = d->d_dec_coef;
        Q.dec_hfscale = d->d_dec_hfscale; Q.dec_state = d->d_dec_state; Q.temp = d->d_temp;
        Q.frames = frames; Q.cd = dd.dry_channels; Q.dec_ir = d->dec_ir;
        Q.real_left = dd.real_left; Q.real_right = dd.real_right; Q.dry_active = d->dry_active;
        if(d->dry_active)
        {
            k_post_hrtf_split<<<dd.dry_channels, 32, 0, d->stream>>>(Q);
            ++d->launches;
        }
        Q.overwrite = d->real_overwrite ? 1u : 0u;
        k_post_hrtf_mix<<<dim3((frames + kHrirLen + 127)/128, 2), 128, 0, d->stream>>>(Q);
        ++d->launches;
        d->carry_idx ^= 1;
        break;
    }
    case B200MIX_POST_AMBIDEC:
    {
        PostAmbiParams Q{};
        Q.dry = d->d_dry; Q.real = d->d_real; Q.gains_hf = d->d_amb_hf; Q.gains_lf = d->d_amb_lf;
        Q.split_state = d->d_amb_state; Q.temp_hf = d->d_temp; Q.temp_lf = d->d_temp2;
// ... 678 lines not shown
```

### openal-soft_b200/csrc/mixer_kernels.cuh

```cuda
#pragma once
#include <cstdint>
#include <cuda_runtime.h>

#include "voice_structs.hpp"
#include "async_ptx.cuh"

namespace b200mix {

constexpr int kLine = 1024;
constexpr int kHrirLen = 128;
constexpr int kHist = 64;
constexpr int kEdge = 24;
constexpr int kPad = 48;
constexpr int kResBuf = kLine + 256 + kPad;
constexpr int kSrcSizeMax = kResBuf - kEdge;
constexpr int kAccumLen = kLine + kHrirLen;
constexpr float kSilence = 0.00001f;
constexpr float kEps = 1.1920929e-07f;

constexpr uint32_t kVfStatic = 1u<<2, kVfLooping = 1u<<3, kVfHrtf = 1u<<4;
constexpr uint32_t kVfFading = 1u<<8, kVfHaveBuffer = 1u<<9, kVfCoefDirty = 1u<<10;
constexpr uint32_t kUpNoBuffer = 1u<<11;
constexpr uint32_t kVfChannelMask = 0xffu<<16;

struct alignas(16) BufferRec {
    const void *data;
    uint32_t frames, type, channels, pad;
};

struct alignas(16) VoiceRec {
    uint32_t state;
    uint32_t flags;
    uint32_t buffer, resampler;
    int32_t  pos; uint32_t frac, step, loop_start;
    uint32_t loop_end; float bsinc_sf; uint32_t bsinc_m, bsinc_l;
    uint32_t bsinc_off, tgt_delay0, tgt_delay1; float tgt_gain;
    uint32_t old_delay0, old_delay1; float old_gain; uint32_t send_mask;
    uint32_t send_slot[kMaxSends]; uint32_t pad2[2];
    float prev[kPad];
    float hist[kHist];
};

struct VoiceResult { int32_t position; uint32_t position_frac, flags, buffers_done; };

struct alignas(16) FilterRec {
    float cur[2][5]; float tgt[2][5];
    float z[2][2];
    int32_t counter[2];
    uint32_t active;
    uint32_t pad[5];
};
static_assert(sizeof(FilterRec) == 128, "FilterRec layout");

struct MixParams {
    VoiceRec *voices; const BufferRec *buffers;
    float2 *hrtf_tgt; float2 *hrtf_old;
    float *dry_cur; float *dry_tgt;
    float *send_cur; float *send_tgt;
    float *dry;
    float *wet;
    float *partial;
    VoiceResult *results;
    const float *bsinc_tab[3];
    const float *cubic_tab[2];
    uint32_t max_voices, frames, ir, ir_pad, cd, cw, num_sends, max_buffers;
    float *xscratch;
    uint32_t *sendinfo;
    const uint32_t *order;
    uint32_t num_order;
    FilterRec *filt;
    uint32_t filt_paths;
    uint32_t pass;
    const float *dline;
    uint4 *qhdr; const uint32_t *queue;
    uint32_t gather_only;
};

constexpr uint32_t kMaxQueue = 32, kNoLoop = 0xffffffffu;

constexpr uint32_t kSiSend = 1u, kSiPlaying = 2u, kSiDeferred = 4u, kSiDirty = 8u, kSiDry = 16u;

__device__ __forceinline__ void group_sync(int id, int count)
{ asm volatile("bar.sync %0, %1;" :: "r"(id), "r"(count) : "memory"); }

__device__ __forceinline__ void prefetch_l2(const void *p)
{ asm volatile("prefetch.global.L2 [%0];" :: "l"(p)); }

__device__ __forceinline__ uint32_t sample_bytes(uint32_t type)
{ return type == 1u ? 2u : ((type == 0u || type >= 5u) ? 1u : (type == 4u ? 8u : 4u)); }

__device__ __forceinline__ void prefetch_span(const char *base, size_t bytes, size_t off,
    size_t len, int t, int gs)
{
    if(off >= bytes) return;
    if(off + len > bytes) len = bytes - off;
    const size_t first = off & ~size_t(127);
    for(size_t a = first + size_t(t)*128u;a < off + len;a += size_t(gs)*128u)
        prefetch_l2(base + a);
}

__device__ __forceinline__ float load_sample(const BufferRec &b, size_t idx)
{
    switch(b.type)
    {
    case 0: return (float(static_cast<const uint8_t*>(b.data)[idx]) - 128.0f) * (1.0f/128.0f);
    case 1: return float(static_cast<const int16_t*>(b.data)[idx]) * (1.0f/32768.0f);
    case 2: return float(static_cast<const int32_t*>(b.data)[idx]) * (1.0f/2147483648.0f);
    case 3: return static_cast<const float*>(b.data)[idx];
    case 4: return float(static_cast<const double*>(b.data)[idx]);
    }
    return 0.0f;
}

__device__ __forceinline__ void calc_buffer_size(uint32_t fracPos, uint32_t increment,
    uint32_t dstRemaining, uint32_t &dst, uint32_t &src)
{
    const uint32_t ext = increment <= 65536u;
    const uint64_t srcSize64 = ((uint64_t(dstRemaining - ext)*increment + fracPos) >> 16)
        + ext + kEdge;
    if(srcSize64 <= uint64_t(kSrcSizeMax)) { dst = dstRemaining; src = uint32_t(srcSize64); return; }
    const uint64_t dstSize64 = ((uint64_t(kSrcSizeMax - kEdge)<<16) - fracPos) / increment;
    if(dstSize64 < dstRemaining) { dst = uint32_t(dstSize64) & ~3u; src = kSrcSizeMax; return; }
    dst = dstRemaining; src = kSrcSizeMax;
}

__device__ __forceinline__ int32_t add_sat(int32_t a, int32_t b)
{
    long long r = (long long)a + b;
    r = r > 2147483647ll ? 2147483647ll : (r < -2147483648ll ? -2147483648ll : r);
    return int32_t(r);
}

__device__ __forceinline__ float to_float(uint8_t v) { return (float(v) - 128.0f) * (1.0f/128.0f); }
__device__ __forceinline__ float to_float(int16_t v) { return float(v) * (1.0f/32768.0f); }
__device__ __forceinline__ float to_float(int32_t v) { return float(v) * (1.0f/2147483648.0f); }
__device__ __forceinline__ float to_float(float v) { return v; }
__device__ __forceinline__ float to_float(double v) { return float(v); }
struct MulawByte { uint8_t v; };
struct AlawByte { uint8_t v; };
__device__ __forceinline__ float to_float(MulawByte b)
{
    const uint32_t u = (~uint32_t(b.v)) & 0xffu;
    const int s = int((((u & 0x0fu)<<3) + 0x84u) << ((u>>4)&7u)) - 0x84;
    return float((u & 0x80u) ? -s : s) * (1.0f/32768.0f);
}
__device__ __forceinline__ float to_float(AlawByte b)
{
    const uint32_t a = uint32_t(b.v) ^ 0x55u;
    const uint32_t e = (a>>4)&7u, m = a & 0x0fu;
    const int s = (e == 0u) ? int((m<<4) + 8u) : int(((m<<4) + 0x108u) << (e-1u));
    return float((a & 0x80u) ? s : -s) * (1.0f/32768.0f);
}

template<typename T> __device__ __forceinline__ T ld_raw(const T *p) { return __ldg(p); }
template<> __device__ __forceinline__ MulawByte ld_raw(const MulawByte *p)
{ return MulawByte{__ldg(reinterpret_cast<const uint8_t*>(p))}; }
template<> __device__ __forceinline__ AlawByte ld_raw(const AlawByte *p)
{ return AlawByte{__ldg(reinterpret_cast<const uint8_t*>(p))}; }

constexpr int kPackB = 688;
static_assert(kPackB >= (kResBuf + 8 + 1)/2 && kPackB + (kResBuf + 8 + 1)/2 <= kResBuf + 8 + 24
    && (kPackB % 32) == 16, "16-bit window copies must fit the float window's storage");

__device__ __forceinline__ float win_at(const float *win, bool packed, uint32_t k)
{
    if(!packed) return win[k];
    const uint16_t y = reinterpret_cast<const uint16_t*>(win)[k];
    return float(int(y) - 32768) * (1.0f/32768.0f);
}

struct FillArgs {
    float *dst; uint32_t count, uintPos, q0, firstRun, loopStart, loopSize, lastFrame, channels;
    bool looping, pastEnd, simpleWrap;
};

__device__ __forceinline__ void filter_clear(FilterRec &fr, int t)
{
    if(t < 10) fr.cur[t/5][t%5] = fr.tgt[t/5][t%5];
    else if(t < 14) fr.z[(t-10)>>1][(t-10)&1] = 0.0f;
    else if(t < 16) fr.counter[t-14] = 0;
}

template<typename T, int GS>
__device__ __forceinline__ void fill_window(const FillArgs &A, const T *__restrict__ src, int t)
{
    for(uint32_t k0 = t;k0 < A.count;k0 += 8u*GS)
    {
        T raw[8];
        #pragma unroll
        for(int u = 0;u < 8;++u)
        {
            uint32_t k = k0 + uint32_t(u)*GS;
            k = k < A.count ? k : A.count-1u;
            uint32_t q;
            if(!A.looping) q = min(A.uintPos + k, A.lastFrame);
            else if(k < A.firstRun) q = A.q0 + k;
            else if(A.simpleWrap) q = A.loopStart + (k - A.firstRun);
            else q = A.loopStart + (k - A.firstRun)%A.loopSize;
            raw[u] = ld_raw(src + size_t(q)*A.channels);
        }
        #pragma unroll
        for(int u = 0;u < 8;++u)
        {
            const uint32_t k = k0 + uint32_t(u)*GS;
            if(k < A.count) A.dst[k] = A.pastEnd ? 0.0f : to_float(raw[u]);
        }
    }
}

template<int GS, int OPT, int FP>
struct alignas(16) GroupSmem {
    static constexpr int kTabStride = kPad + 2;
    static constexpr int kLLen = FP + OPT*GS;
    static constexpr int kOLen = FP + kHist + FP + 32;
    struct ResampleStage { float win[kResBuf + 8 + 24]; alignas(8) float tabF[32*kTabStride]; alignas(8) float tabD[32*kTabStride]; };
    struct FirStage { float2 lLR[kLLen]; float2 oLR[kOLen]; };
    union { ResampleStage rs; FirStage fs; } u;
    float x[kHist + kLine];
    float2 coefT[kHrirLen], coefO[kHrirLen];
    float newGain[32];
    uint64_t tmaBar;
};

__device__ __forceinline__ float2 fma2_rn(float2 a, float2 b, float2 c)
{ return make_float2(__fmaf_rn(a.x, b.x, c.x), __fmaf_rn(a.y, b.y, c.y)); }

template<int OPT, int FP>
__device__ __forceinline__ void fir_pass(float2 (&acc)[OPT], const float2 *__restrict__ in,
    const float2 *__restrict__ coef, int irpad, int t0)
{
    constexpr int JB = 8;
    for(int jb = 0;jb < irpad;jb += JB)
    {
        float2 w[OPT+JB-1];
        const float2 *p = in + FP + t0 - jb - (JB-1);
        #pragma unroll
        for(int k = 0;k < OPT+JB-1;++k) w[k] = p[k];
        #pragma unroll
        for(int jj = 0;jj < JB;++jj)
        {
            const float2 c = coef[jb+jj];
            #pragma unroll
            for(int r = 0;r < OPT;++r)
                acc[r] = fma2_rn(c, w[r - jj + (JB-1)], acc[r]);
        }
    }
}

template<int GS, int GROUPS, bool HRTF, int CDR, int OPT, int FP>
__global__ void __launch_bounds__(GS*GROUPS, GS*GROUPS != 128 ? 1 : ((HRTF || CDR == 0) ? 4 : 3))
k_mix_voices(const MixParams P)
{
    using Smem = GroupSmem<GS, OPT, FP>;
    extern __shared__ __align__(16) unsigned char smem_raw[];
    const int g = threadIdx.x / GS;
    const int t = threadIdx.x % GS;
    Smem &S = reinterpret_cast<Smem*>(smem_raw)[g];
    const int bar = 1 + g;
    constexpr int SPT = kLine / GS;

    float2 acc[OPT];
    #pragma unroll
    for(int r = 0;r < OPT;++r) acc[r] = make_float2(0.0f, 0.0f);
    float accD[CDR > 0 ? CDR : 1][SPT];
    #pragma unroll
    for(int c = 0;c < (CDR > 0 ? CDR : 1);++c)
        #pragma unroll
        for(int r = 0;r < SPT;++r) accD[c][r] = 0.0f;

    const uint32_t n = P.frames;
    const int t0 = OPT*t;
    if(t == 0) { mbar_init(&S.tmaBar, 1u); mbar_fence_init(); }
    uint32_t tmaPhase = 0u;
    group_sync(bar, GS);

    for(uint32_t oi = blockIdx.x*GROUPS + g;oi < P.num_order;oi += gridDim.x*GROUPS)
    {
        const uint32_t v = P.order[oi];
        VoiceRec &rec = P.voices[v];
        const uint4 *hp = reinterpret_cast<const uint4*>(&rec);
        const uint4 h0 = hp[0], h1 = hp[1], h2 = hp[2], h3 = hp[3], h4 = hp[4];
        const bool second = P.pass != 0u;
        uint32_t info = 0u;
        if(second)
        {
            info = P.sendinfo[v];
            if(!(info & kSiDeferred)) continue;
        }
        const uint32_t vstate = second ? ((info & kSiPlaying) ? 1u : 2u) : h0.x;
        if(vstate != 1u && vstate != 2u)
        {
            if(t == 0)
            {
                if(P.results) P.results[v] = VoiceResult{int32_t(h1.x), h1.y, 1u<<7, 0u};
                if(P.sendinfo) P.sendinfo[v] = 0u;
            }
            continue;
        }
        const uint32_t increment = h1.z;
        uint32_t flags = h0.y;
        if(!second && increment < 1u)
        {
            if(t == 0)
            {
                if(vstate == 2u) rec.state = 0u;
                if(P.sendinfo) P.sendinfo[v] = 0u;
                if(P.results)
                    P.results[v] = VoiceResult{int32_t(h1.x), h1.y, (vstate == 2u) ? (1u<<7) : 1u, 0u};
            }
            continue;
        }
        const bool haveBuffer = (flags & kVfHaveBuffer) != 0;
        const BufferRec buf = P.buffers[haveBuffer ? h0.z : 0u];
        const uint32_t loopStart = h1.w, loopEnd = h2.x;
        int32_t intPos = int32_t(h1.x);
        uint32_t fracPos = h1.y;
        bool looping = (flags & kVfLooping) != 0;
        if((flags & kVfStatic) && looping && haveBuffer && intPos >= 0
            && uint32_t(intPos) >= loopEnd)
            looping = false;
        const uint32_t resampler = h0.w;
        const bool isQueue = !(flags & kVfStatic) && P.qhdr != nullptr;
        uint4 qh = make_uint4(0u, 0u, kNoLoop, 0u);
        if(isQueue && !second) qh = P.qhdr[v];
        const uint32_t *qitems = P.queue + size_t(v)*kMaxQueue;
        const bool isHrtf = HRTF && (flags & kVfHrtf);
        const bool dirty = second ? ((info & kSiDirty) != 0) : ((flags & kVfCoefDirty) != 0);
        FilterRec *dfilt = P.filt ? P.filt + size_t(v)*P.filt_paths : nullptr;
        const bool defer = !second && dfilt && dfilt->active;

        if(!second)
            for(int k = t;k < kPad;k += GS) S.u.rs.win[k] = rec.prev[k];
        if(isHrtf && !defer)
        {
            for(int k = t;k < kHist;k += GS) S.x[k] = rec.hist[k];
            const float2 *ct = P.hrtf_tgt + size_t(v)*P.ir_pad;
            const float2 *co = P.hrtf_old + size_t(v)*P.ir_pad;
            for(int k = t;k < int(P.ir_pad);k += GS)
            {
                const float2 c = ct[k];
                S.coefT[k] = c;
                S.coefO[k] = dirty ? co[k] : c;
            }
        }
        uint32_t m = 0, tapOff = 0, ms = 5;
        float *xs = S.x + kHist;
        if(second)
        {
            const float *fl = P.dline + size_t(v)*kLine;
            for(uint32_t k = t;k < n;k += GS) xs[k] = fl[k];
        }
        else
        {
        if(resampler >= 4u)
        {
            m = h2.z;
            tapOff = kEdge - h2.w;
            const float *tab = P.bsinc_tab[(resampler-4u)>>1] + h3.x;
            const bool full = (increment > 65536u) && (resampler & 1u);
            const float sf = __uint_as_float(h2.y);
            const uint32_t rowLen = 2u*m;
            const float *tab2 = tab + 64u*m;
            ms = m + 1u;
            for(uint32_t c = t;c < rowLen;c += GS)
            {
                float *dstc = (c < m) ? (S.u.rs.tabF + c) : (S.u.rs.tabD + (c - m));
                #pragma unroll 1
                for(uint32_t p0 = 0;p0 < 32u;p0 += 8u)
                {
                    float a[8], b[8];
                    #pragma unroll
                    for(int u = 0;u < 8;++u)
                    {
                        a[u] = __ldg(tab + (p0+u)*rowLen + c);
                        b[u] = full ? __ldg(tab2 + (p0+u)*rowLen + c) : 0.0f;
                    }
                    #pragma unroll
                    for(int u = 0;u < 8;++u)
                        dstc[(p0+u)*ms] = full ? fmaf(sf, b[u], a[u]) : a[u];
                }
            }
        }
        else if(resampler >= 2u)
        {
            m = 4; tapOff = kEdge - 1; ms = 5;
            const float *tab = P.cubic_tab[resampler-2u];
            for(uint32_t e = t;e < 128u;e += GS)
            {
                const uint32_t pi = e>>2, j = e&3u;
                S.u.rs.tabF[pi*ms + j] = tab[pi*8u + j];
                S.u.rs.tabD[pi*ms + j] = tab[pi*8u + 4u + j];
            }
        }

        for(uint32_t loaded = 0;loaded < n;)
        {
            uint32_t dstn, srcn;
            calc_buffer_size(fracPos, increment, n-loaded, dstn, srcn);
            uint32_t srcDelay = 0;
            bool silent = false;
            bool packedWin = false;
            if(dstn == 0u) { dstn = n - loaded; silent = true; }
            if(intPos < 0)
            {
                srcDelay = uint32_t(-intPos);
                if(srcDelay >= srcn) silent = true;
            }
            group_sync(bar, GS);
            if(silent)
            {
                for(uint32_t k = t;k < dstn;k += GS) xs[loaded+k] = 0.0f;
                for(uint32_t k = t;k < srcn;k += GS) S.u.rs.win[kEdge+k] = 0.0f;
            }
            else
            {
                float *srcBuffer = S.u.rs.win + kEdge;
                bool winInt = false;
                if(!haveBuffer)
                {
                    const uint32_t avail = srcn < uint32_t(kEdge) ? srcn : uint32_t(kEdge);
                    const uint32_t tofill = srcn > uint32_t(kEdge) ? srcn : uint32_t(kEdge);
                    uint32_t best = 0;
                    for(uint32_t i = 1;i < avail;++i)
                        if(fabsf(srcBuffer[i]) < fabsf(srcBuffer[best])) best = i;
                    const float held = srcBuffer[best];
                    group_sync(bar, GS);
                    for(uint32_t k = best+1+t;k < tofill;k += GS) srcBuffer[k] = held;
                }
                else
                {
                    const uint32_t uintPos = intPos < 0 ? 0u : uint32_t(intPos);
                    const uint32_t count = srcn - srcDelay;
                    float *dst = srcBuffer + srcDelay;
                    for(uint32_t k = t;k < srcDelay;k += GS) srcBuffer[k] = 0.0f;
                    uint32_t done = 0, item = qh.x ? qh.y : kNoLoop, qpos = uintPos;
                    bool more = true;
                    winInt = true;
                    if(!P.gather_only && !isQueue && buf.type == 1u && buf.channels == 1u
                        && ((flags >> 16) & 0xffu) == 0u && count > 0u)
                    {
                        const uint32_t loopSize = looping ? (loopEnd - loopStart) : 1u;
                        const uint32_t q0 = !looping ? uintPos : ((uintPos < loopEnd) ? uintPos
                            : ((uintPos-loopStart)%loopSize + loopStart));
                        const uint32_t run1 = looping ? min(count, loopEnd - q0) : count;
                        const uint32_t run2 = count - run1;
                        const bool fits = looping ? (run2 <= loopSize && loopEnd <= buf.frames)
                                                  : (uintPos + count <= buf.frames);
                        if(fits)
                        {
                            const int16_t *base = static_cast<const int16_t*>(buf.data);
                            const uintptr_t a1 = reinterpret_cast<uintptr_t>(base + q0);
                            const uintptr_t a2 = reinterpret_cast<uintptr_t>(base + loopStart);
                            const uint32_t lead1 = uint32_t(a1 & 15u) >> 1, lead2 = uint32_t(a2 & 15u) >> 1;
                            const uint32_t bytes1 = ((run1 + lead1)*2u + 15u) & ~15u;
                            const uint32_t bytes2 = run2 ? (((run2 + lead2)*2u + 15u) & ~15u) : 0u;
                            constexpr uint32_t kWinBytes = uint32_t(sizeof(S.u.rs.win));
                            unsigned char *wbytes = reinterpret_cast<unsigned char*>(S.u.rs.win);
                            unsigned char *raw2 = wbytes + kWinBytes - bytes2;
                            unsigned char *raw1 = raw2 - bytes1;
                            if(t == 0)
                            {
                                fence_proxy_async_smem();
                                mbar_expect_tx(&S.tmaBar, bytes1 + bytes2);
                                bulk_g2s(raw1, reinterpret_cast<const void*>(a1 & ~uintptr_t(15)), bytes1, &S.tmaBar);
                                if(run2)
                                    bulk_g2s(raw2, reinterpret_cast<const void*>(a2 & ~uintptr_t(15)), bytes2, &S.tmaBar);
                            }
                            mbar_wait(&S.tmaBar, tmaPhase);
                            tmaPhase ^= 1u;
                            const int16_t *r1 = reinterpret_cast<const int16_t*>(raw1) + lead1;
                            const int16_t *r2 = reinterpret_cast<const int16_t*>(raw2) + lead2;
                            constexpr int PERW = (kSrcSizeMax + GS - 1)/GS;
                            float v[PERW];
                            #pragma unroll
                            for(int u = 0;u < PERW;++u)
                            {
                                const uint32_t k = uint32_t(t) + uint32_t(u)*GS;
                                int16_t x = 0;
                                if(k < count) x = k < run1 ? r1[k] : r2[k - run1];
                                v[u] = to_float(x);
                            }
                            group_sync(bar, GS);
                            #pragma unroll
                            for(int u = 0;u < PERW;++u)
                            {
                                const uint32_t k = uint32_t(t) + uint32_t(u)*GS;
                                if(k < count) dst[k] = v[u];
                            }
                            done = count; more = false;
                        }
                    }
                    while(more)
                    {
                        BufferRec rb = buf;
                        FillArgs fa;
                        if(!isQueue)
                        {
                            const uint32_t loopSize = looping ? (loopEnd - loopStart) : 1u;
                            const uint32_t q0 = !looping ? uintPos : ((uintPos < loopEnd) ? uintPos
                                : ((uintPos-loopStart)%loopSize + loopStart));
                            const uint32_t firstRun = looping ? (loopEnd - q0) : 0u;
                            const uint32_t lastFrame = buf.frames ? buf.frames-1u : 0u;
                            const bool pastEnd = !looping && !(buf.frames > uintPos);
                            const bool simpleWrap = looping && count <= firstRun + loopSize;
                            fa = FillArgs{dst, count, uintPos, q0, firstRun, loopStart, loopSize,
                                lastFrame, buf.channels, looping, pastEnd, simpleWrap};
                            done = count; more = false;
                        }
                        else
                        {
                            bool found = false;
                            while(item != kNoLoop && done < count)
                            {
                                rb = P.buffers[qitems[item]];
                                if(qpos >= rb.frames)
                                {
                                    qpos -= rb.frames;
                                    item = (item + 1u < qh.x) ? item + 1u : qh.z;
                                    continue;
                                }
                                found = true;
                                break;
                            }
                            if(!found) break;
                            const uint32_t run = min(count - done, rb.frames - qpos);
                            fa = FillArgs{dst + done, run, qpos, qpos, 0u, 0u, 1u, rb.frames-1u,
                                rb.channels, false, false, false};
                            done += run; qpos = 0u;
                            item = (item + 1u < qh.x) ? item + 1u : qh.z;
                            more = done < count;
                        }
                        winInt = winInt && (rb.type <= 1u || rb.type >= 5u);
                        const uint32_t ch = ((flags >> 16) & 0xffu) < rb.channels ? ((flags >> 16) & 0xffu) : 0u;
                        switch(rb.type)
                        {
                        case 0: fill_window<uint8_t, GS>(fa, static_cast<const uint8_t*>(rb.data) + ch, t); break;
                        case 1: fill_window<int16_t, GS>(fa, static_cast<const int16_t*>(rb.data) + ch, t); break;
                        case 2: fill_window<int32_t, GS>(fa, static_cast<const int32_t*>(rb.data) + ch, t); break;
                        case 3: fill_window<float, GS>(fa, static_cast<const float*>(rb.data) + ch, t); break;
                        case 4: fill_window<double, GS>(fa, static_cast<const double*>(rb.data) + ch, t); break;
                        case 5: fill_window<MulawByte, GS>(fa, static_cast<const MulawByte*>(rb.data) + ch, t); break;
                        default: fill_window<AlawByte, GS>(fa, static_cast<const AlawByte*>(rb.data) + ch, t); break;
                        }
                    }
                    if(done < count)
                    {
                        group_sync(bar, GS);
                        const float held = done ? dst[done-1u] : 0.0f;
                        for(uint32_t k = done + t;k < count;k += GS) dst[k] = held;
                    }
                }
                group_sync(bar, GS);

                packedWin = resampler >= 4u && winInt && !(increment == 65536u && fracPos == 0u);
                if(packedWin)
                {
                    constexpr int PER = (kResBuf + 8 + GS - 1)/GS;
                    const uint32_t L = min(uint32_t(kEdge) + srcn + 8u, uint32_t(kResBuf + 8));
                    float v[PER];
                    #pragma unroll
                    for(int u = 0;u < PER;++u)
                    {
                        const uint32_t k = uint32_t(t) + uint32_t(u)*GS;
                        v[u] = k < L ? S.u.rs.win[k] : 0.0f;
                    }
                    group_sync(bar, GS);
                    uint16_t *pa = reinterpret_cast<uint16_t*>(S.u.rs.win);
                    uint16_t *pb = pa + 2*kPackB;
                    #pragma unroll
                    for(int u = 0;u < PER;++u)
                    {
                        const uint32_t k = uint32_t(t) + uint32_t(u)*GS;
                        if(k < L)
                        {
                            const uint16_t y = uint16_t(__float2int_rn(v[u]*32768.0f) + 32768);
                            pa[k] = y;
                            if(k) pb[k-1u] = y;
                        }
                    }
                    group_sync(bar, GS);
                }

                if(increment == 65536u && fracPos == 0u)
                {
                    for(uint32_t k = t;k < dstn;k += GS) xs[loaded+k] = srcBuffer[k];
                }
                else if(packedWin)
                {
                    const uint32_t *wordsA = reinterpret_cast<const uint32_t*>(S.u.rs.win);
                    const uint32_t *wordsB = wordsA + kPackB;
                    const float2 bias = make_float2(-8421376.0f, -8421376.0f);
                    const float2 one = make_float2(1.0f, 1.0f);
                    for(uint32_t k = t;k < dstn;k += 2u*GS)
                    {
                        const uint32_t kB = k + GS;
                        const bool hasB = kB < dstn;
                        const uint64_t fpA = uint64_t(k)*increment + fracPos;
                        const uint64_t fpB = uint64_t(hasB ? kB : k)*increment + fracPos;
                        const uint32_t fracA = uint32_t(fpA) & 0xffffu, fracB = uint32_t(fpB) & 0xffffu;
                        const float pfA = float(fracA & 2047u) * (1.0f/2048.0f);
                        const float pfB = float(fracB & 2047u) * (1.0f/2048.0f);
                        const float *FA = S.u.rs.tabF + (fracA>>11)*ms, *DA = S.u.rs.tabD + (fracA>>11)*ms;
                        const float *FB = S.u.rs.tabF + (fracB>>11)*ms, *DB = S.u.rs.tabD + (fracB>>11)*ms;
                        const uint32_t posA = tapOff + uint32_t(fpA>>16), posB = tapOff + uint32_t(fpB>>16);
                        const uint32_t *wA = ((posA & 1u) ? wordsB : wordsA) + (posA >> 1);
                        const uint32_t *wB = ((posB & 1u) ? wordsB : wordsA) + (posB >> 1);
                        const float2 pA = make_float2(pfA, pfA), pB = make_float2(pfB, pfB);
                        float2 a0 = make_float2(0.0f, 0.0f), a1 = a0, b0 = a0, b1 = a0;
                        for(uint32_t j = 0;j < m;j += 4)
                        {
                            const uint32_t wa0 = wA[(j>>1)], wa1 = wA[(j>>1)+1u];
                            const uint32_t wb0 = wB[(j>>1)], wb1 = wB[(j>>1)+1u];
                            const float2 sA0 = fma2_rn(make_float2(__uint_as_float(__byte_perm(wa0, 0x4B00u, 0x5410u)),
                                __uint_as_float(__byte_perm(wa0, 0x4B00u, 0x5432u))), one, bias);
                            const float2 sA1 = fma2_rn(make_float2(__uint_as_float(__byte_perm(wa1, 0x4B00u, 0x5410u)),
                                __uint_as_float(__byte_perm(wa1, 0x4B00u, 0x5432u))), one, bias);
                            const float2 sB0 = fma2_rn(make_float2(__uint_as_float(__byte_perm(wb0, 0x4B00u, 0x5410u)),
                                __uint_as_float(__byte_perm(wb0, 0x4B00u, 0x5432u))), one, bias);
                            const float2 sB1 = fma2_rn(make_float2(__uint_as_float(__byte_perm(wb1, 0x4B00u, 0x5410u)),
                                __uint_as_float(__byte_perm(wb1, 0x4B00u, 0x5432u))), one, bias);
                            const float2 cA0 = fma2_rn(pA, make_float2(DA[j+0], DA[j+1]), make_float2(FA[j+0], FA[j+1]));
                            const float2 cB0 = fma2_rn(pB, make_float2(DB[j+0], DB[j+1]), make_float2(FB[j+0], FB[j+1]));
                            const float2 cA1 = fma2_rn(pA, make_float2(DA[j+2], DA[j+3]), make_float2(FA[j+2], FA[j+3]));
                            const float2 cB1 = fma2_rn(pB, make_float2(DB[j+2], DB[j+3]), make_float2(FB[j+2], FB[j+3]));
                            a0 = fma2_rn(cA0, sA0, a0);
                            b0 = fma2_rn(cB0, sB0, b0);
                            a1 = fma2_rn(cA1, sA1, a1);
                            b1 = fma2_rn(cB1, sB1, b1);
                        }
                        xs[loaded+k] = ((a0.x + a1.x) + (a0.y + a1.y)) * (1.0f/32768.0f);
                        if(hasB) xs[loaded+kB] = ((b0.x + b1.x) + (b0.y + b1.y)) * (1.0f/32768.0f);
                    }
                }
                else if(resampler >= 2u)
                {
                    const float *vals = S.u.rs.win + tapOff;
                    for(uint32_t k = t;k < dstn;k += 2u*GS)
                    {
                        const uint32_t kB = k + GS;
                        const bool hasB = kB < dstn;
                        const uint64_t fpA = uint64_t(k)*increment + fracPos;
                        const uint64_t fpB = uint64_t(hasB ? kB : k)*increment + fracPos;
                        const uint32_t fracA = uint32_t(fpA) & 0xffffu, fracB = uint32_t(fpB) & 0xffffu;
                        const float pfA = float(fracA & 2047u) * (1.0f/2048.0f);
                        const float pfB = float(fracB & 2047u) * (1.0f/2048.0f);
                        const float *FA = S.u.rs.tabF + (fracA>>11)*ms, *DA = S.u.rs.tabD + (fracA>>11)*ms;
                        const float *FB = S.u.rs.tabF + (fracB>>11)*ms, *DB = S.u.rs.tabD + (fracB>>11)*ms;
                        const float *svA = vals + uint32_t(fpA>>16), *svB = vals + uint32_t(fpB>>16);
                        const float2 pA = make_float2(pfA, pfA), pB = make_float2(pfB, pfB);
                        float2 a0 = make_float2(0.0f, 0.0f), a1 = a0, b0 = a0, b1 = a0;
                        for(uint32_t j = 0;j < m;j += 4)
                        {
                            const float2 cA0 = fma2_rn(pA, make_float2(DA[j+0], DA[j+1]), make_float2(FA[j+0], FA[j+1]));
                            const float2 cB0 = fma2_rn(pB, make_float2(DB[j+0], DB[j+1]), make_float2(FB[j+0], FB[j+1]));
                            const float2 cA1 = fma2_rn(pA, make_float2(DA[j+2], DA[j+3]), make_float2(FA[j+2], FA[j+3]));
                            const float2 cB1 = fma2_rn(pB, make_float2(DB[j+2], DB[j+3]), make_float2(FB[j+2], FB[j+3]));
                            a0 = fma2_rn(cA0, make_float2(svA[j+0], svA[j+1]), a0);
                            b0 = fma2_rn(cB0, make_float2(svB[j+0], svB[j+1]), b0);
                            a1 = fma2_rn(cA1, make_float2(svA[j+2], svA[j+3]), a1);
                            b1 = fma2_rn(cB1, make_float2(svB[j+2], svB[j+3]), b1);
                        }
                        xs[loaded+k] = (a0.x + a1.x) + (a0.y + a1.y);
                        if(hasB) xs[loaded+kB] = (b0.x + b1.x) + (b0.y + b1.y);
                    }
                }
                else
                {
                    const float *vals = srcBuffer;
                    for(uint32_t k = t;k < dstn;k += GS)
                    {
                        const uint64_t fp = uint64_t(k)*increment + fracPos;
                        const uint32_t pos = uint32_t(fp>>16), frac = uint32_t(fp) & 0xffffu;
                        if(resampler == 0u) xs[loaded+k] = vals[pos];
                        else
                        {
                            const float a = vals[pos], b = vals[pos+1];
                            xs[loaded+k] = a + (b-a)*(float(frac)*(1.0f/65536.0f));
                        }
                    }
                }
            }

            const uint32_t loadEnd = loaded + dstn;
            if(!silent && vstate == 1u && n > loaded && n <= loadEnd)
            {
                const uint32_t dstOffset = n - loaded;
                const uint32_t srcOffset = uint32_t((uint64_t(dstOffset)*increment + fracPos) >> 16);
                for(int k = t;k < kPad;k += GS) rec.prev[k] = win_at(S.u.rs.win, packedWin, srcOffset + uint32_t(k));
            }
            loaded = loadEnd;
            if(loaded < n)
            {
                fracPos += dstn*increment;
                const uint32_t srcOffset = fracPos >> 16;
                fracPos &= 0xffffu;
                if(silent) intPos = add_sat(intPos, int32_t(srcOffset));
                else
                {
                    if(intPos < 0) intPos += int32_t(srcOffset);
                    else intPos = add_sat(intPos, int32_t(srcOffset));
                    float carry = 0.0f;
                    if(t < kPad) carry = win_at(S.u.rs.win, packedWin, srcOffset + uint32_t(t));
                    float carry2 = 0.0f;
                    if(GS < kPad && t + GS < kPad) carry2 = win_at(S.u.rs.win, packedWin, srcOffset + uint32_t(t) + GS);
                    group_sync(bar, GS);
                    if(t < kPad) S.u.rs.win[t] = carry;
                    if(GS < kPad && t + GS < kPad) S.u.rs.win[t + GS] = carry2;
                }
            }
        }
        }
        group_sync(bar, GS);

        const bool fading = (flags & kVfFading) != 0;
        const uint32_t counter = second ? ((info >> 8) & 0xffu) : (fading ? (n < 64u ? n : 64u) : 0u);
        const bool playing = vstate == 1u;

        const bool parkDry = CDR == 0 && !isHrtf;
        if(P.sendinfo && !second)
        {
            const bool sends = P.num_sends && h4.w;
            if(sends || defer || parkDry)
                for(uint32_t k = t;k < n;k += GS) P.xscratch[size_t(v)*kLine + k] = xs[k];
            if(t == 0)
                P.sendinfo[v] = (sends || defer || parkDry) ? ((sends ? kSiSend : 0u)
                    | (playing ? kSiPlaying : 0u) | (defer ? kSiDeferred : 0u) | (dirty ? kSiDirty : 0u)
                    | (parkDry ? kSiDry : 0u) | (counter << 8)) : 0u;
        }
        if(dfilt && !second && !defer) filter_clear(*dfilt, t);

        if(!defer && !parkDry)
        {
        if(isHrtf)
        {
            if(playing)
                for(int k = t;k < kHist;k += GS) rec.hist[k] = S.x[n + k];
            uint32_t oD0 = h4.x, oD1 = h4.y;
            float oGain = __uint_as_float(h4.z);
            const uint32_t tD0 = h3.y, tD1 = h3.z;
            const float tgtGain = __uint_as_float(h3.w);
            if(!counter) { oD0 = tD0; oD1 = tD1; oGain = tgtGain; }
            const bool sameFilter = !counter || (!dirty && oD0 == tD0 && oD1 == tD1);
            const float targetGain = tgtGain * (playing ? 1.0f : 0.0f);
            const uint32_t fademix = counter;
            float blendNewStep = 0.0f, oldStep = 0.0f;
            bool oldOn = false, newOn = false;
            float gainA = oGain;
            if(fademix)
            {
                const float gain = targetGain;
                blendNewStep = gain / float(fademix);
                oldStep = oGain / float(fademix);
                oldOn = oGain > kSilence;
                newOn = blendNewStep*float(fademix) > kSilence;
                gainA = gain;
            }
            const uint32_t todo = n - fademix;
            const float step2 = todo ? (targetGain - gainA) / float(todo) : 0.0f;

            const float *hs = S.x;
            for(int i = t;i < Smem::kLLen;i += GS)
            {
                const int s = i - FP;
                float l = 0.0f, r = 0.0f;
                if(s >= 0 && s < int(n))
                {
                    float gnew;
                    if(uint32_t(s) < fademix)
                        gnew = (newOn && s >= 1) ? blendNewStep*float(s) : 0.0f;
                    else
                        gnew = gainA + step2*float(uint32_t(s) - fademix);
                    l = hs[kHist - tD0 + s] * gnew;
                    r = hs[kHist - tD1 + s] * gnew;
                    if(sameFilter && oldOn && uint32_t(s) < fademix)
                    {
                        const float gold = oldStep*float(fademix - uint32_t(s));
                        l += hs[kHist - oD0 + s] * gold;
                        r += hs[kHist - oD1 + s] * gold;
                    }
                }
                S.u.fs.lLR[i] = make_float2(l, r);
            }
            const bool oldPass = !sameFilter && oldOn;
            if(oldPass)
                for(int i = t;i < Smem::kOLen;i += GS)
                {
                    const int s = i - FP;
                    float l = 0.0f, r = 0.0f;
                    if(s >= 0 && uint32_t(s) < fademix)
                    {
                        const float gold = oldStep*float(fademix - uint32_t(s));
                        l = hs[kHist - oD0 + s] * gold;
                        r = hs[kHist - oD1 + s] * gold;
                    }
                    S.u.fs.oLR[i] = make_float2(l, r);
                }
            group_sync(bar, GS);

    {
                const uint32_t stride = gridDim.x*GROUPS;
                const uint32_t o2 = oi + 2u*stride, o1 = oi + stride;
                const uint32_t v2 = o2 < P.num_order ? P.order[o2] : 0xffffffffu;
                const uint32_t v1 = o1 < P.num_order ? P.order[o1] : 0xffffffffu;
                if(v2 < P.max_voices)
                {
                    if(t < 5) prefetch_l2(reinterpret_cast<const char*>(&P.voices[v2]) + t*128);
                    else if(HRTF && t < 5 + int((P.ir_pad*8u + 127u)/128u))
                        prefetch_l2(reinterpret_cast<const char*>(P.hrtf_tgt + size_t(v2)*P.ir_pad) + (t-5)*128);
                }
                if(v1 < P.max_voices)
                {
                    const VoiceRec &nx = P.voices[v1];
                    if((nx.state == 1u || nx.state == 2u) && (nx.flags & kVfHaveBuffer) && nx.step >= 1u)
                    {
                        const BufferRec nb = P.buffers[nx.buffer];
                        const size_t fb = size_t(sample_bytes(nb.type))*nb.channels;
                        const size_t bytes = size_t(nb.frames)*fb;
                        const uint32_t p0 = nx.pos < 0 ? 0u : uint32_t(nx.pos);
                        const size_t need = size_t((uint64_t(P.frames)*nx.step + nx.frac) >> 16) + kPad;
                        const char *base = static_cast<const char*>(nb.data);
                        prefetch_span(base, bytes, size_t(p0)*fb, need*fb, t, GS);
                        if((nx.flags & kVfLooping) && p0 + need > nx.loop_end && nx.loop_end > p0)
                            prefetch_span(base, bytes, size_t(nx.loop_start)*fb,
                                (p0 + need - nx.loop_end)*fb, t, GS);
                    }
                }
            }
            const int irpad = int(P.ir_pad);
            fir_pass<OPT, FP>(acc, S.u.fs.lLR, S.coefT, irpad, t0);
            if(oldPass && t0 < int(kHist) + irpad)
                fir_pass<OPT, FP>(acc, S.u.fs.oLR, S.coefO, irpad, t0);
            if(t == 0)
            {
                rec.old_delay0 = tD0; rec.old_delay1 = tD1;
                rec.old_gain = targetGain;
            }
        }
        else
        {
            const uint32_t cd = P.cd;
            const float delta = counter ? 1.0f/float(counter) : 0.0f;
            const uint32_t fadeLen = counter < n ? counter : n;
            float *cur = P.dry_cur + size_t(v)*cd;
            const float *tgt = P.dry_tgt + size_t(v)*cd;
            for(uint32_t c = 0;c < cd;++c)
            {
                const float cg = counter ? cur[c] : tgt[c];
                const float tg = playing ? tgt[c] : 0.0f;
                const float step = (tg - cg)*delta;
                const bool fade = fabsf(step) > kEps;
                const bool early = fade && fadeLen < counter;
                const float flat = (!early && fabsf(tg) > kSilence) ? tg : 0.0f;
                const uint32_t start = fade ? fadeLen : 0u;
                #pragma unroll
                for(int r = 0;r < SPT;++r)
                {
                    const uint32_t i = t + r*GS;
                    float gsel = 0.0f;
                    if(i < n)
                        gsel = (fade && i < fadeLen) ? (cg + step*float(i)) : (i >= start ? flat : 0.0f);
                    const float val = xs[i < n ? i : 0]*gsel;
                    if(CDR > 0 && c < uint32_t(CDR))
                    {
                        #pragma unroll
                        for(int cc = 0;cc < (CDR > 0 ? CDR : 1);++cc)
                            if(cc == int(c)) accD[cc][r] += val;
                    }

                }
                if(t == 0)
                    S.newGain[c] = early ? (cg + step*float(fadeLen)) : tg;
            }
        }

        }

        if(t == 0 && !second)
        {
            uint32_t newFlags = (flags | kVfFading) & ~kVfCoefDirty;
            uint32_t newState = vstate;
            uint32_t buffersDone = 0u;
            int32_t pos = int32_t(h1.x); uint32_t frac = h1.y;
            if(vstate == 2u) newState = 0u;
            else
            {
                frac += increment*n;
                const uint32_t done = frac >> 16;
                pos = add_sat(pos, int32_t(done));
                frac &= 0xffffu;
                if(haveBuffer && pos > 0 && isQueue)
                {
                    uint32_t item = qh.x ? qh.y : kNoLoop;
                    while(item != kNoLoop)
                    {
                        const uint32_t len = P.buffers[qitems[item]].frames;
                        if(len > uint32_t(pos)) break;
                        pos -= int32_t(len);
                        ++buffersDone;
                        item = (item + 1u < qh.x) ? item + 1u : qh.z;
                    }
                    if(item == kNoLoop) { newFlags &= ~kVfHaveBuffer; newState = 2u; }
                    else if(item != qh.y) P.qhdr[v].y = item;
                }
                else if(haveBuffer && pos > 0)
                {
                    if(looping)
                    {
                        uint32_t up = uint32_t(pos);
                        if(up >= loopEnd)
                            pos = int32_t((up-loopStart)%(loopEnd-loopStart) + loopStart);
                    }
                    else if(uint32_t(pos) >= buf.frames)
                    {
                        newFlags &= ~kVfHaveBuffer;
                        newState = 2u;
                    }
                }
                rec.pos = pos; rec.frac = frac;
            }
            rec.flags = newFlags;
            rec.state = newState;
            if(P.results)
                P.results[v] = VoiceResult{pos, frac,
                    newState == 1u ? 1u : (newState == 2u ? 2u : (1u<<7)), buffersDone};
        }
        group_sync(bar, GS);
        if(t == 0)
        {
            if(!isHrtf && !defer && !parkDry)
                for(uint32_t c = 0;c < P.cd;++c)
                    P.dry_cur[size_t(v)*P.cd + c] = S.newGain[c];
        }
        group_sync(bar, GS);
    }

    const size_t row = blockIdx.x;
    __syncthreads();
    float *stage = reinterpret_cast<float*>(smem_raw);
    if(HRTF)
    {
        for(int gg = 0;gg < GROUPS;++gg)
        {
            if(g == gg)
            {
                #pragma unroll
                for(int r = 0;r < OPT;++r)
                {
                    const int o = t0 + r;
                    if(o < kAccumLen)
                    {
                        if(gg == 0) { stage[o] = acc[r].x; stage[kAccumLen + o] = acc[r].y; }
                        else { stage[o] += acc[r].x; stage[kAccumLen + o] += acc[r].y; }
                    }
                }
                if(gg == 0 && GS*OPT < kAccumLen)
                    for(int o = GS*OPT + t;o < kAccumLen;o += GS) { stage[o] = 0.0f; stage[kAccumLen + o] = 0.0f; }
            }
            __syncthreads();
        }
        float *pl = P.partial + row*(2*kAccumLen);
        for(int o = threadIdx.x;o < 2*kAccumLen;o += GS*GROUPS) pl[o] = stage[o];
        __syncthreads();
    }
    if(CDR > 0)
    {
        const size_t rows = gridDim.x;
        float *pd = P.partial + (HRTF ? rows*(2*kAccumLen) : 0) + row*(size_t(CDR)*kLine);
        if(GROUPS == 1)
        {
            #pragma unroll
            for(int c = 0;c < (CDR > 0 ? CDR : 1);++c)
                #pragma unroll
                for(int r = 0;r < SPT;++r)
                    pd[c*kLine + t + r*GS] = accD[c][r];
        }
        else
        {
            for(int gg = 0;gg < GROUPS;++gg)
            {
                if(g == gg)
                {
                    #pragma unroll
                    for(int c = 0;c < (CDR > 0 ? CDR : 1);++c)
                        #pragma unroll
                        for(int r = 0;r < SPT;++r)
                        {
                            float *dst = stage + c*kLine + t + r*GS;
                            if(gg == 0) *dst = accD[c][r]; else *dst += accD[c][r];
                        }
                }
                __syncthreads();
            }
            for(int o = threadIdx.x;o < CDR*kLine;o += GS*GROUPS) pd[o] = stage[o];
        }
    }
}

constexpr int kReduceCols = 8, kReduceSegs = 128;
__global__ void __launch_bounds__(1024)
k_reduce_rows(const float *__restrict__ partial, uint32_t rows, uint32_t len,
    float *__restrict__ out, int accumulate)
{
    __shared__ float4 sm[kReduceSegs][kReduceCols];
    const uint32_t col = threadIdx.x & (kReduceCols-1), seg = threadIdx.x / kReduceCols;
    const uint32_t e4 = blockIdx.x*kReduceCols + col;
    float4 s = make_float4(0.f, 0.f, 0.f, 0.f);
    if(e4*4u < len)
    {
        const uint32_t per = (rows + kReduceSegs - 1u)/kReduceSegs;
        const uint32_t r0 = seg*per, r1 = (r0 + per < rows) ? r0 + per : rows;
        const float4 *p = reinterpret_cast<const float4*>(partial) + e4;
        const size_t stride4 = len/4u;
        uint32_t r = r0;
        for(;r + 4u <= r1;r += 4u)
        {
            const float4 a = __ldg(p + size_t(r)*stride4), b = __ldg(p + size_t(r+1)*stride4);
            const float4 c = __ldg(p + size_t(r+2)*stride4), d = __ldg(p + size_t(r+3)*stride4);
            s.x += a.x; s.y += a.y; s.z += a.z; s.w += a.w;
            s.x += b.x; s.y += b.y; s.z += b.z; s.w += b.w;
            s.x += c.x; s.y += c.y; s.z += c.z; s.w += c.w;
            s.x += d.x; s.y += d.y; s.z += d.z; s.w += d.w;
        }
        for(;r < r1;++r)
        {
            const float4 a = __ldg(p + size_t(r)*stride4);
            s.x += a.x; s.y += a.y; s.z += a.z; s.w += a.w;
        }
    }
    sm[seg][col] = s;
    __syncthreads();
    #pragma unroll
    for(uint32_t width = kReduceSegs/4u;width >= 1u;width /= 4u)
    {
        float4 tot = make_float4(0.f, 0.f, 0.f, 0.f);
        const bool on = seg < width;
        if(on)
        {
            tot = sm[seg*4u][col];
            #pragma unroll
            for(uint32_t k = 1;k < 4u;++k)
            {
                const float4 a = sm[seg*4u + k][col];
                tot.x += a.x; tot.y += a.y; tot.z += a.z; tot.w += a.w;
            }
        }
        __syncthreads();
        if(on) sm[seg][col] = tot;
        __syncthreads();
        if(width == 2u) break;
    }
    if(seg == 0 && e4*4u < len)
    {
        float4 tot = sm[0][col];
        const float4 b = sm[1][col];
        tot.x += b.x; tot.y += b.y; tot.z += b.z; tot.w += b.w;
        float4 *o = reinterpret_cast<float4*>(out) + e4;
        if(accumulate)
        {
            const float4 a = *o;
            tot.x += a.x; tot.y += a.y; tot.z += a.z; tot.w += a.w;
        }
        *o = tot;
    }
}

__global__ void __launch_bounds__(256)
k_reduce_few(const float *__restrict__ partial, uint32_t rows, uint32_t len,
    float *__restrict__ out, int accumulate)
{
    const uint32_t e4 = blockIdx.x*blockDim.x + threadIdx.x;
    if(e4*4u >= len) return;
    const float4 *p = reinterpret_cast<const float4*>(partial) + e4;
    const size_t stride4 = len/4u;
    float4 v[16];
    #pragma unroll
    for(uint32_t r = 0;r < 16u;++r)
        v[r] = r < rows ? __ldg(p + size_t(r)*stride4) : make_float4(0.f, 0.f, 0.f, 0.f);
    float4 g[4];
    #pragma unroll
    for(uint32_t j = 0;j < 4u;++j)
    {
        float4 t = v[4u*j];
        #pragma unroll
        for(uint32_t k = 1;k < 4u;++k)
        { t.x += v[4u*j+k].x; t.y += v[4u*j+k].y; t.z += v[4u*j+k].z; t.w += v[4u*j+k].w; }
        g[j] = t;
    }
    float4 tot = g[0];
    #pragma unroll
    for(uint32_t j = 1;j < 4u;++j) { tot.x += g[j].x; tot.y += g[j].y; tot.z += g[j].z; tot.w += g[j].w; }
    float4 *o = reinterpret_cast<float4*>(out) + e4;
    if(accumulate)
    {
        const float4 a = *o;
        tot.x += a.x; tot.y += a.y; tot.z += a.z; tot.w += a.w;
    }
    *o = tot;
}

struct ApplyParams {
    VoiceRec *voices; const VoiceUpdate *updates;
    const float *coeffs; const float *dry; const float *send;
    float2 *hrtf_tgt; float2 *hrtf_old; float *dry_cur, *dry_tgt, *send_cur, *send_tgt;
    uint32_t ir, ir_pad, cd, cw, num_sends;
    FilterRec *filt; uint32_t filt_paths;
    const float4 *dirs;
    const float2 *st_fields;
    const uint2 *st_elevs;
    const float2 *st_coeffs;
    const uint8_t *st_delays;
    uint32_t st_num_fields, st_ir;
    uint4 *qhdr;
};

struct HrirBlend { uint32_t idx[4]; float w[4]; float passthru; uint32_t delay[2]; };

__device__ __forceinline__ void hrir_index(uint32_t count, float v, bool elev, uint32_t &idx, float &blend)
{
    const float inv_pi = 0.318309886183790671538f;
    if(elev)
    {
        v = __fmul_rn(__fadd_rn(__fmul_rn(inv_pi, v), 0.5f), float(count-1u));
        const uint32_t i = v > 0.0f ? uint32_t(v) : 0u;
        idx = min(i, count-1u); blend = __fsub_rn(v, float(i));
    }
    else
    {
        v = __fmul_rn(__fadd_rn(__fmul_rn(inv_pi*0.5f, v), 1.0f), float(count));
        const uint32_t i = v > 0.0f ? uint32_t(v) : 0u;
        idx = i % count; blend = __fsub_rn(v, float(i));
    }
}

__device__ __forceinline__ void hrir_blend(const ApplyParams &A, const float4 dir, HrirBlend &B)
{
    const float inv_pi = 0.318309886183790671538f;
    const float elevation = dir.x, azimuth = dir.y, distance = dir.z, spread = dir.w;
    const float dirfact = __fsub_rn(1.0f, __fmul_rn(inv_pi/2.0f, spread));
    uint32_t ebase = 0, fi = 0;
    for(;fi + 1u < A.st_num_fields;++fi)
    {
        if(distance >= A.st_fields[fi].x) break;
        ebase += __float_as_uint(A.st_fields[fi].y);
    }
    const uint32_t evCount = __float_as_uint(A.st_fields[fi].y);
    uint32_t e0i; float e0b;
    hrir_index(evCount, elevation, true, e0i, e0b);
    const uint32_t e1i = min(e0i + 1u, evCount - 1u);
    const uint2 el0 = A.st_elevs[ebase + e0i], el1 = A.st_elevs[ebase + e1i];
    uint32_t a0i, a1i; float a0b, a1b;
    hrir_index(el0.x, azimuth, false, a0i, a0b);
    hrir_index(el1.x, azimuth, false, a1i, a1b);
    B.idx[0] = el0.y + a0i; B.idx[1] = el0.y + ((a0i + 1u) % el0.x);
    B.idx[2] = el1.y + a1i; B.idx[3] = el1.y + ((a1i + 1u) % el1.x);
    const float ne = __fsub_rn(1.0f, e0b);
    B.w[0] = __fmul_rn(__fmul_rn(ne, __fsub_rn(1.0f, a0b)), dirfact);
    B.w[1] = __fmul_rn(__fmul_rn(ne, a0b), dirfact);
    B.w[2] = __fmul_rn(__fmul_rn(e0b, __fsub_rn(1.0f, a1b)), dirfact);
    B.w[3] = __fmul_rn(__fmul_rn(e0b, a1b), dirfact);
    #pragma unroll
    for(int ear = 0;ear < 2;++ear)
    {
        float dsum = __fmul_rn(float(A.st_delays[B.idx[0]*2u + ear]), B.w[0]);
        dsum = __fadd_rn(dsum, __fmul_rn(float(A.st_delays[B.idx[1]*2u + ear]), B.w[1]));
        dsum = __fadd_rn(dsum, __fmul_rn(float(A.st_delays[B.idx[2]*2u + ear]), B.w[2]));
        dsum = __fadd_rn(dsum, __fmul_rn(float(A.st_delays[B.idx[3]*2u + ear]), B.w[3]));
        B.delay[ear] = uint32_t(__float2int_rn(__fmul_rn(dsum, 0.25f)));
    }
    B.passthru = __fmul_rn(0.70710678118654752440f, __fsub_rn(1.0f, dirfact));
}

__device__ __forceinline__ void filter_reset_word(FilterRec *fr, int k)
{
    uint32_t *w = reinterpret_cast<uint32_t*>(fr);
    uint32_t val = 0u;
    if(k == 0 || k == 5 || k == 10 || k == 15) val = __float_as_uint(1.0f);
    else if(k == 24 || k == 25) val = 0xffffffffu;
    w[k] = val;
}

struct QueueSet { uint32_t voice, count, loop; uint32_t items[kMaxQueue]; };
__global__ void k_set_queue(VoiceRec *voices, uint4 *qhdr, uint32_t *queue, const QueueSet Q)
{
    const uint32_t t = threadIdx.x;
    if(t < Q.count) queue[size_t(Q.voice)*kMaxQueue + t] = Q.items[t];
    if(t == 0)
    {
        qhdr[Q.voice] = make_uint4(Q.count, 0u, Q.loop, 0u);
        uint32_t fl = voices[Q.voice].flags;
        fl = Q.count ? (fl | kVfHaveBuffer) : (fl & ~kVfHaveBuffer);
        voices[Q.voice].flags = fl;
    }
}

__global__ void k_filter_init(FilterRec *filt, size_t count)
{
    const size_t i = size_t(blockIdx.x)*blockDim.x + threadIdx.x;
    if(i < count*32u) filter_reset_word(filt + (i >> 5), int(i & 31u));
}

__global__ void k_apply_filter_updates(FilterRec *filt, uint32_t paths, const FilterUpdate *upd,
    uint32_t n)
{
    const uint32_t i = blockIdx.x*blockDim.x + threadIdx.x;
    if(i >= n*2u) return;
    const FilterUpdate &u = upd[i >> 1];
    const int f = int(i & 1u);
    FilterRec &fr = filt[size_t(u.voice)*paths + u.path];
    const float *nt = f ? u.hp : u.lp;
    bool diff = false;
    #pragma unroll
    for(int k = 0;k < 5;++k)
    {
        diff |= !(fabsf(nt[k] - fr.tgt[f][k]) <= 0.015625f);
        fr.tgt[f][k] = nt[k];
    }
    const int c = fr.counter[f];
    if(!diff)
    {
        if(c <= 0)
        {
            fr.counter[f] = 0;
            #pragma unroll
            for(int k = 0;k < 5;++k) fr.cur[f][k] = nt[k];
        }
    }
    else if(c >= 0) fr.counter[f] = 8*32;
    else
    {
        fr.counter[f] = 0;
        #pragma unroll
        for(int k = 0;k < 5;++k) fr.cur[f][k] = nt[k];
    }
    if(f == 0) fr.active = u.active ? 1u : 0u;
}

__global__ void __launch_bounds__(64) k_apply_updates(const ApplyParams A)
{
    const uint32_t u = blockIdx.x;
    const VoiceUpdate up = A.updates[u];
    VoiceRec &rec = A.voices[up.voice];
    const int t = threadIdx.x;
    const bool reset = (up.flags & (1u<<5)) != 0;
    const uint32_t oldFlags = reset ? 0u : rec.flags;
    const bool wasDirty = (oldFlags & kVfCoefDirty) != 0;
    __syncthreads();
    if(reset)
    {
        for(int k = t;k < kPad;k += 64) rec.prev[k] = 0.0f;
        for(int k = t;k < kHist;k += 64) rec.hist[k] = 0.0f;
        if(A.dry_cur) for(uint32_t c = t;c < A.cd;c += 64) A.dry_cur[size_t(up.voice)*A.cd + c] = 0.0f;
        if(A.send_cur)
            for(uint32_t c = t;c < A.num_sends*A.cw;c += 64)
                A.send_cur[size_t(up.voice)*A.num_sends*A.cw + c] = 0.0f;
        if(A.filt)
            for(uint32_t k = t;k < A.filt_paths*32u;k += 64)
                filter_reset_word(A.filt + size_t(up.voice)*A.filt_paths + (k >> 5), int(k & 31u));
    }
    __shared__ HrirBlend sB;
    const bool fromDirs = A.dirs != nullptr && up.has_coeffs && A.hrtf_tgt;
    if(fromDirs)
    {
        if(t == 0) hrir_blend(A, A.dirs[u], sB);
        __syncthreads();
    }
    if(up.has_coeffs && A.hrtf_tgt)
    {
        float2 *tg = A.hrtf_tgt + size_t(up.voice)*A.ir_pad;
        float2 *ol = A.hrtf_old + size_t(up.voice)*A.ir_pad;
        const float *src = fromDirs ? nullptr : A.coeffs + size_t(u)*A.ir*2;
        for(uint32_t k = t;k < A.ir_pad;k += 64)
        {
            if(!wasDirty && !reset) ol[k] = tg[k];
            float2 val = make_float2(0.f, 0.f);
            if(fromDirs)
            {
                if(k < A.st_ir && k < A.ir)
                {
                    val = (k == 0) ? make_float2(sB.passthru, sB.passthru) : val;
                    #pragma unroll
                    for(int c = 0;c < 4;++c)
                    {
                        const float2 sv = A.st_coeffs[size_t(sB.idx[c])*A.st_ir + k];
                        val.x = __fadd_rn(__fmul_rn(sv.x, sB.w[c]), val.x);
                        val.y = __fadd_rn(__fmul_rn(sv.y, sB.w[c]), val.y);
                    }
                }
            }
            else if(k < A.ir) val = make_float2(src[k*2], src[k*2+1]);
            tg[k] = val;
        }
    }
    if(up.has_dry && A.dry_tgt)
        for(uint32_t c = t;c < A.cd;c += 64)
            A.dry_tgt[size_t(up.voice)*A.cd + c] = A.dry[size_t(u)*A.cd + c];
    if(A.send && A.send_tgt)
        for(uint32_t c = t;c < A.num_sends*A.cw;c += 64)
            A.send_tgt[size_t(up.voice)*A.num_sends*A.cw + c] = A.send[size_t(u)*A.num_sends*A.cw + c];
    if(t == 0)
// ... 845 lines not shown
```

Baseline: 27.01 billion.

## Split HRTF FIR out of the voice mixer into a dedicated kernel

Result: faster. 28.44 billion (median of 6 runs) (+5.3%).

```diff
diff --git a/openal-soft_b200/csrc/b200mix.cu b/openal-soft_b200/csrc/b200mix.cu
--- a/openal-soft_b200/csrc/b200mix.cu
+++ b/openal-soft_b200/csrc/b200mix.cu
@@ -199,6 +199,8 @@
     int mix_variant{0}; int mix_groups{2}; int mix_gs{64}; int mix_cdr{0};
     uint32_t reverb_seq{0};
     size_t mix_smem{0}; int mix_blocks_per_sm{1};
+    uint32_t *d_claim{nullptr};
+    int fir_blocks_per_sm{0};
 };
 
 namespace {
@@ -218,24 +220,25 @@
 
 using MixKernel = void(*)(const MixParams);
 
-struct Variant { MixKernel fn; int gs, groups, cdr; size_t smem; bool hrtf; };
-
-template<int GS, int GROUPS, bool HRTF, int CDR, int OPT, int FP>
+struct Variant { MixKernel fn; int gs, groups, cdr; size_t smem; };
+
+template<int GS, int GROUPS, int CDR>
 Variant make_variant()
 {
-    return Variant{k_mix_voices<GS, GROUPS, HRTF, CDR, OPT, FP>, GS, GROUPS, CDR,
-        sizeof(GroupSmem<GS, OPT, FP>)*GROUPS, HRTF};
+    return Variant{k_mix_voices<GS, GROUPS, CDR>, GS, GROUPS, CDR, sizeof(GroupSmem<CDR>)*GROUPS};
 }
 
 Variant get_variant(int idx)
 {
-    switch(idx)
-    {
-    case 0: return make_variant<64, 2, true, 0, 17, 64>();
-    case 1: return make_variant<64, 2, true, 0, 19, 128>();
-    case 2: return make_variant<64, 2, false, 4, 1, 8>();
-    default: return make_variant<64, 2, false, 0, 1, 8>();
-    }
+    return idx == 0 ? make_variant<64, 2, 4>() : make_variant<64, 2, 0>();
+}
+
+struct FirVariant { MixKernel fn; size_t smem; };
+FirVariant get_fir(uint32_t ir_size)
+{
+    if(ir_size <= 64u)
+        return FirVariant{k_hrtf_fir<17, 64>, sizeof(FirSmem<kFirGS, 17, 64>)*kFirGroups};
+    return FirVariant{k_hrtf_fir<19, 128>, sizeof(FirSmem<kFirGS, 19, 128>)*kFirGroups};
 }
 
 constexpr uint32_t kDryChunksMax = 128;
@@ -389,13 +392,26 @@
         d->h_hrtf.assign(dd.max_voices, 0);
 
         const bool hrtfDev = dd.ir_size > 0;
-        d->mix_variant = hrtfDev ? (dd.ir_size <= 64 ? 0 : 1) : (dd.dry_channels <= 4 ? 2 : 3);
+        d->mix_variant = (!hrtfDev && dd.dry_channels <= 4) ? 0 : 1;
         const Variant var = get_variant(d->mix_variant);
         d->mix_gs = var.gs; d->mix_groups = var.groups; d->mix_cdr = var.cdr; d->mix_smem = var.smem;
         CUDA_TRY(d, cudaFuncSetAttribute(var.fn, cudaFuncAttributeMaxDynamicSharedMemorySize, int(var.smem)));
         int perSm = 0;
         CUDA_TRY(d, cudaOccupancyMaxActiveBlocksPerMultiprocessor(&perSm, var.fn, var.gs*var.groups, var.smem));
         d->mix_blocks_per_sm = std::max(perSm, 1);
+        if(var.cdr == 0)
+        {
+            if(int rc = dev_alloc(d, d->d_xscratch, size_t(dd.max_voices)*kLine)) return rc;
+            if(int rc = dev_alloc(d, d->d_sendinfo, dd.max_voices)) return rc;
+            if(int rc = dev_alloc(d, d->d_claim, 2)) return rc;
+        }
+        if(hrtfDev)
+        {
+            const FirVariant fir = get_fir(dd.ir_size);
+            CUDA_TRY(d, cudaFuncSetAttribute(fir.fn, cudaFuncAttributeMaxDynamicSharedMemorySize, int(fir.smem)));
+            CUDA_TRY(d, cudaOccupancyMaxActiveBlocksPerMultiprocessor(&perSm, fir.fn, kFirGS*kFirGroups, fir.smem));
+            d->fir_blocks_per_sm = std::max(std::min(perSm, kFirCtasPerSm), 1);
+        }
 
         d->dry_alloc_ch = std::max<uint32_t>(std::max(dd.dry_channels, 1u), uint32_t(var.cdr));
         if(int rc = dev_alloc(d, d->d_dry, size_t(d->dry_alloc_ch)*kLine)) return rc;
@@ -416,9 +432,9 @@
         }
         if(dd.max_slots && dd.wet_channels)
             if(int rc = dev_alloc(d, d->d_wet, size_t(dd.max_slots)*dd.wet_channels*kLine)) return rc;
-        const size_t maxRows = size_t(d->num_sms)*d->mix_blocks_per_sm;
-        d->partial_floats = maxRows*(hrtfDev ? 2*kAccumLen : 0) + maxRows*size_t(var.cdr)*kLine;
-        if(int rc = dev_alloc(d, d->d_partial, std::max<size_t>(2*d->partial_floats, 4))) return rc;
+        d->partial_floats = hrtfDev ? size_t(d->num_sms)*d->fir_blocks_per_sm*(2*kAccumLen)
+            : size_t(d->num_sms)*d->mix_blocks_per_sm*size_t(var.cdr)*kLine;
+        if(int rc = dev_alloc(d, d->d_partial, std::max<size_t>((hrtfDev ? 1 : 2)*d->partial_floats, 4))) return rc;
         if(int rc = dev_alloc(d, d->d_accum_sum, 2*kAccumLen)) return rc;
         if(int rc = dev_alloc(d, d->d_carry[0], 2*kHrirLen)) return rc;
         if(int rc = dev_alloc(d, d->d_carry[1], 2*kHrirLen)) return rc;
@@ -429,8 +445,10 @@
             d->h_slots.assign(dd.max_slots, SlotRec{});
             d->slot_allocs.assign(dd.max_slots, {});
             if(int rc = dev_alloc(d, d->d_slots, dd.max_slots)) return rc;
-            if(int rc = dev_alloc(d, d->d_xscratch, size_t(dd.max_voices)*kLine)) return rc;
-            if(int rc = dev_alloc(d, d->d_sendinfo, dd.max_voices)) return rc;
+            if(!d->d_xscratch)
+                if(int rc = dev_alloc(d, d->d_xscratch, size_t(dd.max_voices)*kLine)) return rc;
+            if(!d->d_sendinfo)
+                if(int rc = dev_alloc(d, d->d_sendinfo, dd.max_voices)) return rc;
             if(int rc = dev_alloc(d, d->d_send_geff, size_t(dd.max_voices)*dd.num_sends*dd.wet_channels)) return rc;
             if(int rc = dev_alloc(d, d->d_send_gramp, size_t(dd.max_voices)*dd.num_sends*dd.wet_channels)) return rc;
             d->h_send_slot.assign(size_t(dd.max_voices)*B200MIX_MAX_SENDS, B200MIX_NO_SLOT);
@@ -488,7 +506,7 @@
     cudaFree(d->d_uhj_state); cudaFree(d->d_uhj_scratch);
     cudaFree(d->d_uhj_fir_state); cudaFree(d->d_uhj_fir_coef); cudaFree(d->d_bs2b); cudaFree(d->d_stab_state);
     for(auto &v : d->slot_allocs) for(void *p : v) cudaFree(p);
-    cudaFree(d->d_slots); cudaFree(d->d_xscratch); cudaFree(d->d_sendinfo);
+    cudaFree(d->d_slots); cudaFree(d->d_xscratch); cudaFree(d->d_sendinfo); cudaFree(d->d_claim);
     cudaFree(d->d_filt); cudaFree(d->d_fupd); cudaFree(d->d_fscratch);
     cudaFree(d->d_dline); cudaFree(d->d_order2); cudaFree(d->d_qhdr); cudaFree(d->d_queue);
     cudaFree(d->d_outbuf); if(d->h_outbuf) cudaFreeHost(d->h_outbuf);
@@ -1646,10 +1664,10 @@
         d->order2_dirty = false;
     }
     const Variant var = get_variant(d->mix_variant);
+    const bool hrtfDev = dd.ir_size > 0;
     const uint32_t nv = std::max(d->voice_hi, 1u);
     const uint32_t maxBlocks = uint32_t(d->num_sms*d->mix_blocks_per_sm);
     const uint32_t blocks = std::max(1u, std::min(maxBlocks, (d->num_order + var.groups - 1)/var.groups));
-    const size_t rows = size_t(blocks);
 
     MixParams P{};
     P.voices = d->d_voices; P.buffers = d->d_buffers;
@@ -1668,10 +1686,11 @@
     P.filt = d->d_filt; P.filt_paths = 1u + dd.num_sends;
     P.qhdr = d->d_qhdr; P.queue = d->d_queue;
     P.gather_only = d->mix_gather_only ? 1u : 0u;
+    P.claim = d->d_claim;
+    P.dline = d->d_dline;
     stage_mark(d, 1);
     if(d->profile) cudaEventRecord(d->ev_mix0, d->stream);
     var.fn<<<blocks, var.gs*var.groups, var.smem, d->stream>>>(P);
-    if(d->profile) { cudaEventRecord(d->ev_mix1, d->stream); d->ev_valid = true; }
     ++d->launches;
     CUDA_TRY(d, cudaGetLastError());
 
@@ -1685,42 +1704,49 @@
         FP.xscratch = d->d_xscratch; FP.dline = d->d_dline; FP.frames = frames;
         k_filters<<<(d->num_order2 + 31u)/32u, 32, 0, d->stream>>>(FP);
         ++d->launches;
-        const uint32_t blocks2 = std::max(1u, std::min(maxBlocks, (d->num_order2 + var.groups - 1)/var.groups));
-        rows2 = blocks2;
-        MixParams P2 = P;
-        P2.pass = 1u; P2.dline = d->d_dline;
-        P2.order = d->d_order2; P2.num_order = d->num_order2;
-        P2.partial = d->d_partial + d->partial_floats;
-        P2.results = nullptr;
-        var.fn<<<blocks2, var.gs*var.groups, var.smem, d->stream>>>(P2);
+        if(var.cdr > 0)
+        {
+            const uint32_t blocks2 = std::max(1u, std::min(maxBlocks, (d->num_order2 + var.groups - 1)/var.groups));
+            rows2 = blocks2;
+            MixParams P2 = P;
+            P2.pass = 1u;
+            P2.order = d->d_order2; P2.num_order = d->num_order2;
+            P2.partial = d->d_partial + d->partial_floats;
+            P2.results = nullptr;
+            var.fn<<<blocks2, var.gs*var.groups, var.smem, d->stream>>>(P2);
+            ++d->launches;
+        }
+        CUDA_TRY(d, cudaGetLastError());
+    }
+    uint32_t firBlocks = 0;
+    if(hrtfDev)
+    {
+        const FirVariant fir = get_fir(dd.ir_size);
+        firBlocks = std::max(1u, std::min(uint32_t(d->num_sms*d->fir_blocks_per_sm),
+            (d->num_order + kFirGroups - 1)/kFirGroups));
+        fir.fn<<<firBlocks, kFirGS*kFirGroups, fir.smem, d->stream>>>(P);
         ++d->launches;
         CUDA_TRY(d, cudaGetLastError());
     }
+    if(d->profile) { cudaEventRecord(d->ev_mix1, d->stream); d->ev_valid = true; }
 
     stage_mark(d, 3);
-    if(var.hrtf)
+    if(hrtfDev)
     {
         const uint32_t len = 2*kAccumLen;
-        k_reduce_rows<<<(len/4 + kReduceCols - 1)/kReduceCols, 1024, 0, d->stream>>>(d->d_partial, uint32_t(rows), len,
+        k_reduce_rows<<<(len/4 + kReduceCols - 1)/kReduceCols, 1024, 0, d->stream>>>(d->d_partial, firBlocks, len,
             d->d_accum_sum, 0);
         ++d->launches;
-        if(rows2)
-        {
-            k_reduce_rows<<<(len/4 + kReduceCols - 1)/kReduceCols, 1024, 0, d->stream>>>(d->d_partial + d->partial_floats,
-                uint32_t(rows2), len, d->d_accum_sum, 1);
-            ++d->launches;
-        }
     }
     if(var.cdr > 0)
     {
         const uint32_t len = uint32_t(var.cdr)*kLine;
-        const float *pd = d->d_partial + (var.hrtf ? rows*(2*kAccumLen) : 0);
-        k_reduce_rows<<<(len/4 + kReduceCols - 1)/kReduceCols, 1024, 0, d->stream>>>(pd, uint32_t(rows), len, d->d_dry, 1);
+        k_reduce_rows<<<(len/4 + kReduceCols - 1)/kReduceCols, 1024, 0, d->stream>>>(d->d_partial, blocks, len, d->d_dry, 1);
         ++d->launches;
         if(rows2)
         {
-            const float *pd2 = d->d_partial + d->partial_floats + (var.hrtf ? rows2*(2*kAccumLen) : 0);
-            k_reduce_rows<<<(len/4 + kReduceCols - 1)/kReduceCols, 1024, 0, d->stream>>>(pd2, uint32_t(rows2), len, d->d_dry, 1);
+            k_reduce_rows<<<(len/4 + kReduceCols - 1)/kReduceCols, 1024, 0, d->stream>>>(d->d_partial + d->partial_floats,
+                uint32_t(rows2), len, d->d_dry, 1);
             ++d->launches;
         }
     }
diff --git a/openal-soft_b200/csrc/mixer_kernels.cuh b/openal-soft_b200/csrc/mixer_kernels.cuh
--- a/openal-soft_b200/csrc/mixer_kernels.cuh
+++ b/openal-soft_b200/csrc/mixer_kernels.cuh
@@ -74,14 +74,19 @@
     const float *dline;
     uint4 *qhdr; const uint32_t *queue;
     uint32_t gather_only;
+    uint32_t *claim;
 };
 
 constexpr uint32_t kMaxQueue = 32, kNoLoop = 0xffffffffu;
 
-constexpr uint32_t kSiSend = 1u, kSiPlaying = 2u, kSiDeferred = 4u, kSiDirty = 8u, kSiDry = 16u;
+constexpr uint32_t kSiSend = 1u, kSiPlaying = 2u, kSiDeferred = 4u, kSiDirty = 8u, kSiDry = 16u,
+    kSiHrtf = 32u;
 
 __device__ __forceinline__ void group_sync(int id, int count)
-{ asm volatile("bar.sync %0, %1;" :: "r"(id), "r"(count) : "memory"); }
+{
+    if(id == 1) asm volatile("bar.sync 1, %0;" :: "r"(count) : "memory");
+    else asm volatile("bar.sync 2, %0;" :: "r"(count) : "memory");
+}
 
 __device__ __forceinline__ void prefetch_l2(const void *p)
 { asm volatile("prefetch.global.L2 [%0];" :: "l"(p)); }
@@ -208,18 +213,26 @@
     }
 }
 
-template<int GS, int OPT, int FP>
+template<int CDR>
 struct alignas(16) GroupSmem {
     static constexpr int kTabStride = kPad + 2;
+    float win[kResBuf + 8 + 24];
+    alignas(8) float tabF[32*kTabStride];
+    alignas(8) float tabD[32*kTabStride];
+    float x[CDR > 0 ? kLine : 1];
+    float newGain[32];
+    uint64_t tmaBar;
+    uint32_t claimed;
+};
+
+template<int GS, int OPT, int FP>
+struct alignas(16) FirSmem {
     static constexpr int kLLen = FP + OPT*GS;
     static constexpr int kOLen = FP + kHist + FP + 32;
-    struct ResampleStage { float win[kResBuf + 8 + 24]; alignas(8) float tabF[32*kTabStride]; alignas(8) float tabD[32*kTabStride]; };
-    struct FirStage { float2 lLR[kLLen]; float2 oLR[kOLen]; };
-    union { ResampleStage rs; FirStage fs; } u;
+    float2 lLR[kLLen];
+    float2 oLR[kOLen];
     float x[kHist + kLine];
     float2 coefT[kHrirLen], coefO[kHrirLen];
-    float newGain[32];
-    uint64_t tmaBar;
 };
 
 __device__ __forceinline__ float2 fma2_rn(float2 a, float2 b, float2 c)
@@ -247,11 +260,29 @@
     }
 }
 
-template<int GS, int GROUPS, bool HRTF, int CDR, int OPT, int FP>
-__global__ void __launch_bounds__(GS*GROUPS, GS*GROUPS != 128 ? 1 : ((HRTF || CDR == 0) ? 4 : 3))
+__device__ __forceinline__ uint32_t claim_voice(const MixParams &P, uint32_t &slot, int t, int bar,
+    int gs, uint32_t groups)
+{
+    group_sync(bar, gs);
+    if(t == 0)
+    {
+        uint32_t oi = atomicAdd(P.claim, 1u);
+        if(oi >= P.num_order && atomicAdd(P.claim + 1, 1u) == groups - 1u)
+        {
+            atomicExch(P.claim, 0u);
+            atomicExch(P.claim + 1, 0u);
+        }
+        slot = oi;
+    }
+    group_sync(bar, gs);
+    return slot;
+}
+
+template<int GS, int GROUPS, int CDR>
+__global__ void __launch_bounds__(GS*GROUPS, GS*GROUPS != 128 ? 1 : (CDR == 0 ? 5 : 3))
 k_mix_voices(const MixParams P)
 {
-    using Smem = GroupSmem<GS, OPT, FP>;
+    using Smem = GroupSmem<CDR>;
     extern __shared__ __align__(16) unsigned char smem_raw[];
     const int g = threadIdx.x / GS;
     const int t = threadIdx.x % GS;
@@ -259,9 +290,6 @@
     const int bar = 1 + g;
     constexpr int SPT = kLine / GS;
 
-    float2 acc[OPT];
-    #pragma unroll
-    for(int r = 0;r < OPT;++r) acc[r] = make_float2(0.0f, 0.0f);
     float accD[CDR > 0 ? CDR : 1][SPT];
     #pragma unroll
     for(int c = 0;c < (CDR > 0 ? CDR : 1);++c)
@@ -269,12 +297,14 @@
         for(int r = 0;r < SPT;++r) accD[c][r] = 0.0f;
 
     const uint32_t n = P.frames;
-    const int t0 = OPT*t;
     if(t == 0) { mbar_init(&S.tmaBar, 1u); mbar_fence_init(); }
     uint32_t tmaPhase = 0u;
     group_sync(bar, GS);
 
-    for(uint32_t oi = blockIdx.x*GROUPS + g;oi < P.num_order;oi += gridDim.x*GROUPS)
+    const uint32_t groups = gridDim.x*GROUPS;
+    for(uint32_t oi = CDR > 0 ? blockIdx.x*GROUPS + g : claim_voice(P, S.claimed, t, bar, GS, groups);
+        oi < P.num_order;
+        oi = CDR > 0 ? oi + groups : claim_voice(P, S.claimed, t, bar, GS, groups))
     {
         const uint32_t v = P.order[oi];
         VoiceRec &rec = P.voices[v];
@@ -324,27 +354,15 @@
         uint4 qh = make_uint4(0u, 0u, kNoLoop, 0u);
         if(isQueue && !second) qh = P.qhdr[v];
         const uint32_t *qitems = P.queue + size_t(v)*kMaxQueue;
-        const bool isHrtf = HRTF && (flags & kVfHrtf);
+        const bool isHrtf = CDR == 0 && P.ir_pad != 0u && (flags & kVfHrtf);
         const bool dirty = second ? ((info & kSiDirty) != 0) : ((flags & kVfCoefDirty) != 0);
         FilterRec *dfilt = P.filt ? P.filt + size_t(v)*P.filt_paths : nullptr;
         const bool defer = !second && dfilt && dfilt->active;
 
         if(!second)
-            for(int k = t;k < kPad;k += GS) S.u.rs.win[k] = rec.prev[k];
-        if(isHrtf && !defer)
-        {
-            for(int k = t;k < kHist;k += GS) S.x[k] = rec.hist[k];
-            const float2 *ct = P.hrtf_tgt + size_t(v)*P.ir_pad;
-            const float2 *co = P.hrtf_old + size_t(v)*P.ir_pad;
-            for(int k = t;k < int(P.ir_pad);k += GS)
-            {
-                const float2 c = ct[k];
-                S.coefT[k] = c;
-                S.coefO[k] = dirty ? co[k] : c;
-            }
-        }
+            for(int k = t;k < kPad;k += GS) S.win[k] = rec.prev[k];
         uint32_t m = 0, tapOff = 0, ms = 5;
-        float *xs = S.x + kHist;
+        float *xs = CDR > 0 ? S.x : P.xscratch + size_t(v)*kLine;
         if(second)
         {
             const float *fl = P.dline + size_t(v)*kLine;
@@ -364,7 +382,7 @@
             ms = m + 1u;
             for(uint32_t c = t;c < rowLen;c += GS)
             {
-                float *dstc = (c < m) ? (S.u.rs.tabF + c) : (S.u.rs.tabD + (c - m));
+                float *dstc = (c < m) ? (S.tabF + c) : (S.tabD + (c - m));
                 #pragma unroll 1
                 for(uint32_t p0 = 0;p0 < 32u;p0 += 8u)
                 {
@@ -388,8 +406,34 @@
             for(uint32_t e = t;e < 128u;e += GS)
             {
                 const uint32_t pi = e>>2, j = e&3u;
-                S.u.rs.tabF[pi*ms + j] = tab[pi*8u + j];
-                S.u.rs.tabD[pi*ms + j] = tab[pi*8u + 4u + j];
+                S.tabF[pi*ms + j] = tab[pi*8u + j];
+                S.tabD[pi*ms + j] = tab[pi*8u + 4u + j];
+            }
+        }
+
+        if(CDR == 0)
+        {
+            const uint32_t o2 = oi + 2u*groups, o1 = oi + groups;
+            const uint32_t v2 = o2 < P.num_order ? P.order[o2] : 0xffffffffu;
+            const uint32_t v1 = o1 < P.num_order ? P.order[o1] : 0xffffffffu;
+            if(v2 < P.max_voices && t < 5)
+                prefetch_l2(reinterpret_cast<const char*>(&P.voices[v2]) + t*128);
+            if(v1 < P.max_voices)
+            {
+                const VoiceRec &nx = P.voices[v1];
+                if((nx.state == 1u || nx.state == 2u) && (nx.flags & kVfHaveBuffer) && nx.step >= 1u)
+                {
+                    const BufferRec nb = P.buffers[nx.buffer];
+                    const size_t fb = size_t(sample_bytes(nb.type))*nb.channels;
+                    const size_t bytes = size_t(nb.frames)*fb;
+                    const uint32_t p0 = nx.pos < 0 ? 0u : uint32_t(nx.pos);
+                    const size_t need = size_t((uint64_t(P.frames)*nx.step + nx.frac) >> 16) + kPad;
+                    const char *base = static_cast<const char*>(nb.data);
+                    prefetch_span(base, bytes, size_t(p0)*fb, need*fb, t, GS);
+                    if((nx.flags & kVfLooping) && p0 + need > nx.loop_end && nx.loop_end > p0)
+                        prefetch_span(base, bytes, size_t(nx.loop_start)*fb,
+                            (p0 + need - nx.loop_end)*fb, t, GS);
+                }
             }
         }
 
@@ -410,11 +454,11 @@
             if(silent)
             {
                 for(uint32_t k = t;k < dstn;k += GS) xs[loaded+k] = 0.0f;
-                for(uint32_t k = t;k < srcn;k += GS) S.u.rs.win[kEdge+k] = 0.0f;
+                for(uint32_t k = t;k < srcn;k += GS) S.win[kEdge+k] = 0.0f;
             }
             else
             {
-                float *srcBuffer = S.u.rs.win + kEdge;
+                float *srcBuffer = S.win + kEdge;
                 bool winInt = false;
                 if(!haveBuffer)
                 {
@@ -454,8 +498,8 @@
                             const uint32_t lead1 = uint32_t(a1 & 15u) >> 1, lead2 = uint32_t(a2 & 15u) >> 1;
                             const uint32_t bytes1 = ((run1 + lead1)*2u + 15u) & ~15u;
                             const uint32_t bytes2 = run2 ? (((run2 + lead2)*2u + 15u) & ~15u) : 0u;
-                            constexpr uint32_t kWinBytes = uint32_t(sizeof(S.u.rs.win));
-                            unsigned char *wbytes = reinterpret_cast<unsigned char*>(S.u.rs.win);
+                            constexpr uint32_t kWinBytes = uint32_t(sizeof(S.win));
+                            unsigned char *wbytes = reinterpret_cast<unsigned char*>(S.win);
                             unsigned char *raw2 = wbytes + kWinBytes - bytes2;
                             unsigned char *raw1 = raw2 - bytes1;
                             if(t == 0)
@@ -562,10 +606,10 @@
                     for(int u = 0;u < PER;++u)
                     {
                         const uint32_t k = uint32_t(t) + uint32_t(u)*GS;
-                        v[u] = k < L ? S.u.rs.win[k] : 0.0f;
+                        v[u] = k < L ? S.win[k] : 0.0f;
                     }
                     group_sync(bar, GS);
-                    uint16_t *pa = reinterpret_cast<uint16_t*>(S.u.rs.win);
+                    uint16_t *pa = reinterpret_cast<uint16_t*>(S.win);
                     uint16_t *pb = pa + 2*kPackB;
                     #pragma unroll
                     for(int u = 0;u < PER;++u)
@@ -587,7 +631,7 @@
                 }
                 else if(packedWin)
                 {
-                    const uint32_t *wordsA = reinterpret_cast<const uint32_t*>(S.u.rs.win);
+                    const uint32_t *wordsA = reinterpret_cast<const uint32_t*>(S.win);
                     const uint32_t *wordsB = wordsA + kPackB;
                     const float2 bias = make_float2(-8421376.0f, -8421376.0f);
                     const float2 one = make_float2(1.0f, 1.0f);
@@ -600,8 +644,8 @@
                         const uint32_t fracA = uint32_t(fpA) & 0xffffu, fracB = uint32_t(fpB) & 0xffffu;
                         const float pfA = float(fracA & 2047u) * (1.0f/2048.0f);
                         const float pfB = float(fracB & 2047u) * (1.0f/2048.0f);
-                        const float *FA = S.u.rs.tabF + (fracA>>11)*ms, *DA = S.u.rs.tabD + (fracA>>11)*ms;
-                        const float *FB = S.u.rs.tabF + (fracB>>11)*ms, *DB = S.u.rs.tabD + (fracB>>11)*ms;
+                        const float *FA = S.tabF + (fracA>>11)*ms, *DA = S.tabD + (fracA>>11)*ms;
+                        const float *FB = S.tabF + (fracB>>11)*ms, *DB = S.tabD + (fracB>>11)*ms;
                         const uint32_t posA = tapOff + uint32_t(fpA>>16), posB = tapOff + uint32_t(fpB>>16);
                         const uint32_t *wA = ((posA & 1u) ? wordsB : wordsA) + (posA >> 1);
                         const uint32_t *wB = ((posB & 1u) ? wordsB : wordsA) + (posB >> 1);
@@ -634,7 +678,7 @@
                 }
                 else if(resampler >= 2u)
                 {
-                    const float *vals = S.u.rs.win + tapOff;
+                    const float *vals = S.win + tapOff;
                     for(uint32_t k = t;k < dstn;k += 2u*GS)
                     {
                         const uint32_t kB = k + GS;
@@ -644,8 +688,8 @@
                         const uint32_t fracA = uint32_t(fpA) & 0xffffu, fracB = uint32_t(fpB) & 0xffffu;
                         const float pfA = float(fracA & 2047u) * (1.0f/2048.0f);
                         const float pfB = float(fracB & 2047u) * (1.0f/2048.0f);
-                        const float *FA = S.u.rs.tabF + (fracA>>11)*ms, *DA = S.u.rs.tabD + (fracA>>11)*ms;
-                        const float *FB = S.u.rs.tabF + (fracB>>11)*ms, *DB = S.u.rs.tabD + (fracB>>11)*ms;
+                        const float *FA = S.tabF + (fracA>>11)*ms, *DA = S.tabD + (fracA>>11)*ms;
+                        const float *FB = S.tabF + (fracB>>11)*ms, *DB = S.tabD + (fracB>>11)*ms;
                         const float *svA = vals + uint32_t(fpA>>16), *svB = vals + uint32_t(fpB>>16);
                         const float2 pA = make_float2(pfA, pfA), pB = make_float2(pfB, pfB);
                         float2 a0 = make_float2(0.0f, 0.0f), a1 = a0, b0 = a0, b1 = a0;
@@ -686,7 +730,7 @@
             {
                 const uint32_t dstOffset = n - loaded;
                 const uint32_t srcOffset = uint32_t((uint64_t(dstOffset)*increment + fracPos) >> 16);
-                for(int k = t;k < kPad;k += GS) rec.prev[k] = win_at(S.u.rs.win, packedWin, srcOffset + uint32_t(k));
+                for(int k = t;k < kPad;k += GS) rec.prev[k] = win_at(S.win, packedWin, srcOffset + uint32_t(k));
             }
             loaded = loadEnd;
             if(loaded < n)
@@ -700,12 +744,12 @@
                     if(intPos < 0) intPos += int32_t(srcOffset);
                     else intPos = add_sat(intPos, int32_t(srcOffset));
                     float carry = 0.0f;
-                    if(t < kPad) carry = win_at(S.u.rs.win, packedWin, srcOffset + uint32_t(t));
+                    if(t < kPad) carry = win_at(S.win, packedWin, srcOffset + uint32_t(t));
                     float carry2 = 0.0f;
-                    if(GS < kPad && t + GS < kPad) carry2 = win_at(S.u.rs.win, packedWin, srcOffset + uint32_t(t) + GS);
+                    if(GS < kPad && t + GS < kPad) carry2 = win_at(S.win, packedWin, srcOffset + uint32_t(t) + GS);
                     group_sync(bar, GS);
-                    if(t < kPad) S.u.rs.win[t] = carry;
-                    if(GS < kPad && t + GS < kPad) S.u.rs.win[t + GS] = carry2;
+                    if(t < kPad) S.win[t] = carry;
+                    if(GS < kPad && t + GS < kPad) S.win[t + GS] = carry2;
                 }
             }
         }
@@ -716,163 +760,54 @@
         const uint32_t counter = second ? ((info >> 8) & 0xffu) : (fading ? (n < 64u ? n : 64u) : 0u);
         const bool playing = vstate == 1u;
 
-        const bool parkDry = CDR == 0 && !isHrtf;
         if(P.sendinfo && !second)
         {
             const bool sends = P.num_sends && h4.w;
-            if(sends || defer || parkDry)
+            const bool park = sends || defer || CDR == 0;
+            if(CDR > 0 && park)
                 for(uint32_t k = t;k < n;k += GS) P.xscratch[size_t(v)*kLine + k] = xs[k];
             if(t == 0)
-                P.sendinfo[v] = (sends || defer || parkDry) ? ((sends ? kSiSend : 0u)
+                P.sendinfo[v] = park ? ((sends ? kSiSend : 0u)
                     | (playing ? kSiPlaying : 0u) | (defer ? kSiDeferred : 0u) | (dirty ? kSiDirty : 0u)
-                    | (parkDry ? kSiDry : 0u) | (counter << 8)) : 0u;
+                    | ((CDR == 0 && !isHrtf) ? kSiDry : 0u) | (isHrtf ? kSiHrtf : 0u) | (counter << 8)) : 0u;
         }
         if(dfilt && !second && !defer) filter_clear(*dfilt, t);
 
-        if(!defer && !parkDry)
-        {
-        if(isHrtf)
-        {
-            if(playing)
-                for(int k = t;k < kHist;k += GS) rec.hist[k] = S.x[n + k];
-            uint32_t oD0 = h4.x, oD1 = h4.y;
-            float oGain = __uint_as_float(h4.z);
-            const uint32_t tD0 = h3.y, tD1 = h3.z;
-            const float tgtGain = __uint_as_float(h3.w);
-            if(!counter) { oD0 = tD0; oD1 = tD1; oGain = tgtGain; }
-            const bool sameFilter = !counter || (!dirty && oD0 == tD0 && oD1 == tD1);
-            const float targetGain = tgtGain * (playing ? 1.0f : 0.0f);
-            const uint32_t fademix = counter;
-            float blendNewStep = 0.0f, oldStep = 0.0f;
-            bool oldOn = false, newOn = false;
-            float gainA = oGain;
-            if(fademix)
-            {
-                const float gain = targetGain;
-                blendNewStep = gain / float(fademix);
-                oldStep = oGain / float(fademix);
-                oldOn = oGain > kSilence;
-                newOn = blendNewStep*float(fademix) > kSilence;
-                gainA = gain;
-            }
-            const uint32_t todo = n - fademix;
-            const float step2 = todo ? (targetGain - gainA) / float(todo) : 0.0f;
-
-            const float *hs = S.x;
-            for(int i = t;i < Smem::kLLen;i += GS)
-            {
-                const int s = i - FP;
-                float l = 0.0f, r = 0.0f;
-                if(s >= 0 && s < int(n))
+        if(CDR > 0 && !defer)
+        {
+        const uint32_t cd = P.cd;
+        const float delta = counter ? 1.0f/float(counter) : 0.0f;
+        const uint32_t fadeLen = counter < n ? counter : n;
+        float *cur = P.dry_cur + size_t(v)*cd;
+        const float *tgt = P.dry_tgt + size_t(v)*cd;
+        for(uint32_t c = 0;c < cd;++c)
+        {
+            const float cg = counter ? cur[c] : tgt[c];
+            const float tg = playing ? tgt[c] : 0.0f;
+            const float step = (tg - cg)*delta;
+            const bool fade = fabsf(step) > kEps;
+            const bool early = fade && fadeLen < counter;
+            const float flat = (!early && fabsf(tg) > kSilence) ? tg : 0.0f;
+            const uint32_t start = fade ? fadeLen : 0u;
+            #pragma unroll
+            for(int r = 0;r < SPT;++r)
+            {
+                const uint32_t i = t + r*GS;
+                float gsel = 0.0f;
+                if(i < n)
+                    gsel = (fade && i < fadeLen) ? (cg + step*float(i)) : (i >= start ? flat : 0.0f);
+                const float val = xs[i < n ? i : 0]*gsel;
+                if(CDR > 0 && c < uint32_t(CDR))
                 {
-                    float gnew;
-                    if(uint32_t(s) < fademix)
-                        gnew = (newOn && s >= 1) ? blendNewStep*float(s) : 0.0f;
-                    else
-                        gnew = gainA + step2*float(uint32_t(s) - fademix);
-                    l = hs[kHist - tD0 + s] * gnew;
-                    r = hs[kHist - tD1 + s] * gnew;
-                    if(sameFilter && oldOn && uint32_t(s) < fademix)
-                    {
-                        const float gold = oldStep*float(fademix - uint32_t(s));
-                        l += hs[kHist - oD0 + s] * gold;
-                        r += hs[kHist - oD1 + s] * gold;
-                    }
+                    #pragma unroll
+                    for(int cc = 0;cc < (CDR > 0 ? CDR : 1);++cc)
+                        if(cc == int(c)) accD[cc][r] += val;
                 }
-                S.u.fs.lLR[i] = make_float2(l, r);
-            }
-            const bool oldPass = !sameFilter && oldOn;
-            if(oldPass)
-                for(int i = t;i < Smem::kOLen;i += GS)
-                {
-                    const int s = i - FP;
-                    float l = 0.0f, r = 0.0f;
-                    if(s >= 0 && uint32_t(s) < fademix)
-                    {
-                        const float gold = oldStep*float(fademix - uint32_t(s));
-                        l = hs[kHist - oD0 + s] * gold;
-                        r = hs[kHist - oD1 + s] * gold;
-                    }
-                    S.u.fs.oLR[i] = make_float2(l, r);
-                }
-            group_sync(bar, GS);
-
-    {
-                const uint32_t stride = gridDim.x*GROUPS;
-                const uint32_t o2 = oi + 2u*stride, o1 = oi + stride;
-                const uint32_t v2 = o2 < P.num_order ? P.order[o2] : 0xffffffffu;
-                const uint32_t v1 = o1 < P.num_order ? P.order[o1] : 0xffffffffu;
-                if(v2 < P.max_voices)
-                {
-                    if(t < 5) prefetch_l2(reinterpret_cast<const char*>(&P.voices[v2]) + t*128);
-                    else if(HRTF && t < 5 + int((P.ir_pad*8u + 127u)/128u))
-                        prefetch_l2(reinterpret_cast<const char*>(P.hrtf_tgt + size_t(v2)*P.ir_pad) + (t-5)*128);
-                }
-                if(v1 < P.max_voices)
-                {
-                    const VoiceRec &nx = P.voices[v1];
-                    if((nx.state == 1u || nx.state == 2u) && (nx.flags & kVfHaveBuffer) && nx.step >= 1u)
-                    {
-                        const BufferRec nb = P.buffers[nx.buffer];
-                        const size_t fb = size_t(sample_bytes(nb.type))*nb.channels;
-                        const size_t bytes = size_t(nb.frames)*fb;
-                        const uint32_t p0 = nx.pos < 0 ? 0u : uint32_t(nx.pos);
-                        const size_t need = size_t((uint64_t(P.frames)*nx.step + nx.frac) >> 16) + kPad;
-                        const char *base = static_cast<const char*>(nb.data);
-                        prefetch_span(base, bytes, size_t(p0)*fb, need*fb, t, GS);
-                        if((nx.flags & kVfLooping) && p0 + need > nx.loop_end && nx.loop_end > p0)
-                            prefetch_span(base, bytes, size_t(nx.loop_start)*fb,
-                                (p0 + need - nx.loop_end)*fb, t, GS);
-                    }
-                }
-            }
-            const int irpad = int(P.ir_pad);
-            fir_pass<OPT, FP>(acc, S.u.fs.lLR, S.coefT, irpad, t0);
-            if(oldPass && t0 < int(kHist) + irpad)
-                fir_pass<OPT, FP>(acc, S.u.fs.oLR, S.coefO, irpad, t0);
+
+            }
             if(t == 0)
-            {
-                rec.old_delay0 = tD0; rec.old_delay1 = tD1;
-                rec.old_gain = targetGain;
-            }
-        }
-        else
-        {
-            const uint32_t cd = P.cd;
-            const float delta = counter ? 1.0f/float(counter) : 0.0f;
-            const uint32_t fadeLen = counter < n ? counter : n;
-            float *cur = P.dry_cur + size_t(v)*cd;
-            const float *tgt = P.dry_tgt + size_t(v)*cd;
-            for(uint32_t c = 0;c < cd;++c)
-            {
-                const float cg = counter ? cur[c] : tgt[c];
-                const float tg = playing ? tgt[c] : 0.0f;
-                const float step = (tg - cg)*delta;
-                const bool fade = fabsf(step) > kEps;
-                const bool early = fade && fadeLen < counter;
-                const float flat = (!early && fabsf(tg) > kSilence) ? tg : 0.0f;
-                const uint32_t start = fade ? fadeLen : 0u;
-                #pragma unroll
-                for(int r = 0;r < SPT;++r)
-                {
-                    const uint32_t i = t + r*GS;
-                    float gsel = 0.0f;
-                    if(i < n)
-                        gsel = (fade && i < fadeLen) ? (cg + step*float(i)) : (i >= start ? flat : 0.0f);
-                    const float val = xs[i < n ? i : 0]*gsel;
-                    if(CDR > 0 && c < uint32_t(CDR))
-                    {
-                        #pragma unroll
-                        for(int cc = 0;cc < (CDR > 0 ? CDR : 1);++cc)
-                            if(cc == int(c)) accD[cc][r] += val;
-                    }
-
-                }
-                if(t == 0)
-                    S.newGain[c] = early ? (cg + step*float(fadeLen)) : tg;
-            }
-        }
-
+                S.newGain[c] = early ? (cg + step*float(fadeLen)) : tg;
+        }
         }
 
         if(t == 0 && !second)
@@ -927,45 +862,19 @@
         group_sync(bar, GS);
         if(t == 0)
         {
-            if(!isHrtf && !defer && !parkDry)
+            if(CDR > 0 && !defer)
                 for(uint32_t c = 0;c < P.cd;++c)
                     P.dry_cur[size_t(v)*P.cd + c] = S.newGain[c];
         }
         group_sync(bar, GS);
     }
 
-    const size_t row = blockIdx.x;
-    __syncthreads();
-    float *stage = reinterpret_cast<float*>(smem_raw);
-    if(HRTF)
-    {
-        for(int gg = 0;gg < GROUPS;++gg)
-        {
-            if(g == gg)
-            {
-                #pragma unroll
-                for(int r = 0;r < OPT;++r)
-                {
-                    const int o = t0 + r;
-                    if(o < kAccumLen)
-                    {
-                        if(gg == 0) { stage[o] = acc[r].x; stage[kAccumLen + o] = acc[r].y; }
-                        else { stage[o] += acc[r].x; stage[kAccumLen + o] += acc[r].y; }
-                    }
-                }
-                if(gg == 0 && GS*OPT < kAccumLen)
-                    for(int o = GS*OPT + t;o < kAccumLen;o += GS) { stage[o] = 0.0f; stage[kAccumLen + o] = 0.0f; }
-            }
-            __syncthreads();
-        }
-        float *pl = P.partial + row*(2*kAccumLen);
-        for(int o = threadIdx.x;o < 2*kAccumLen;o += GS*GROUPS) pl[o] = stage[o];
+    if(CDR > 0)
+    {
+        const size_t row = blockIdx.x;
         __syncthreads();
-    }
-    if(CDR > 0)
-    {
-        const size_t rows = gridDim.x;
-        float *pd = P.partial + (HRTF ? rows*(2*kAccumLen) : 0) + row*(size_t(CDR)*kLine);
+        float *stage = reinterpret_cast<float*>(smem_raw);
+        float *pd = P.partial + row*(size_t(CDR)*kLine);
         if(GROUPS == 1)
         {
             #pragma unroll
@@ -995,6 +904,173 @@
         }
     }
 }
+
+constexpr int kFirGS = 64, kFirGroups = 2, kFirCtasPerSm = 4;
+
+template<int OPT, int FP>
+__global__ void __launch_bounds__(kFirGS*kFirGroups, kFirCtasPerSm)
+k_hrtf_fir(const MixParams P)
+{
+    constexpr int GS = kFirGS, GROUPS = kFirGroups;
+    using Smem = FirSmem<GS, OPT, FP>;
+    extern __shared__ __align__(16) unsigned char smem_raw[];
+    const int g = threadIdx.x / GS;
+    const int t = threadIdx.x % GS;
+    Smem &S = reinterpret_cast<Smem*>(smem_raw)[g];
+    const int bar = 1 + g;
+    const int t0 = OPT*t;
+    const uint32_t n = P.frames;
+
+    float2 acc[OPT];
+    #pragma unroll
+    for(int r = 0;r < OPT;++r) acc[r] = make_float2(0.0f, 0.0f);
+
+    const uint32_t stride = gridDim.x*GROUPS;
+    for(uint32_t oi = blockIdx.x*GROUPS + g;oi < P.num_order;oi += stride)
+    {
+        const uint32_t v = P.order[oi];
+        const uint32_t info = P.sendinfo[v];
+        if(!(info & kSiHrtf)) continue;
+        VoiceRec &rec = P.voices[v];
+        const uint4 *hp = reinterpret_cast<const uint4*>(&rec);
+        const uint4 h3 = hp[3], h4 = hp[4];
+        const bool playing = (info & kSiPlaying) != 0;
+        const bool dirty = (info & kSiDirty) != 0;
+        const uint32_t counter = (info >> 8) & 0xffu;
+
+        const float *line = ((info & kSiDeferred) ? P.dline : P.xscratch) + size_t(v)*kLine;
+        for(int k = t;k < kHist;k += GS) S.x[k] = rec.hist[k];
+        for(uint32_t k = t;k < n;k += GS) S.x[kHist + k] = line[k];
+        const float2 *ct = P.hrtf_tgt + size_t(v)*P.ir_pad;
+        const float2 *co = P.hrtf_old + size_t(v)*P.ir_pad;
+        for(int k = t;k < int(P.ir_pad);k += GS)
+        {
+            const float2 c = ct[k];
+            S.coefT[k] = c;
+            S.coefO[k] = dirty ? co[k] : c;
+        }
+        group_sync(bar, GS);
+
+
+        if(playing)
+            for(int k = t;k < kHist;k += GS) rec.hist[k] = S.x[n + k];
+        uint32_t oD0 = h4.x, oD1 = h4.y;
+        float oGain = __uint_as_float(h4.z);
+        const uint32_t tD0 = h3.y, tD1 = h3.z;
+        const float tgtGain = __uint_as_float(h3.w);
+        if(!counter) { oD0 = tD0; oD1 = tD1; oGain = tgtGain; }
+        const bool sameFilter = !counter || (!dirty && oD0 == tD0 && oD1 == tD1);
+        const float targetGain = tgtGain * (playing ? 1.0f : 0.0f);
+        const uint32_t fademix = counter;
+        float blendNewStep = 0.0f, oldStep = 0.0f;
+        bool oldOn = false, newOn = false;
+        float gainA = oGain;
+        if(fademix)
+        {
+            const float gain = targetGain;
+            blendNewStep = gain / float(fademix);
+            oldStep = oGain / float(fademix);
+            oldOn = oGain > kSilence;
+            newOn = blendNewStep*float(fademix) > kSilence;
+            gainA = gain;
+        }
+        const uint32_t todo = n - fademix;
+        const float step2 = todo ? (targetGain - gainA) / float(todo) : 0.0f;
+
+        const float *hs = S.x;
+        for(int i = t;i < Smem::kLLen;i += GS)
+        {
+            const int s = i - FP;
+            float l = 0.0f, r = 0.0f;
+            if(s >= 0 && s < int(n))
+            {
+                float gnew;
+                if(uint32_t(s) < fademix)
+                    gnew = (newOn && s >= 1) ? blendNewStep*float(s) : 0.0f;
+                else
+                    gnew = gainA + step2*float(uint32_t(s) - fademix);
+                l = hs[kHist - tD0 + s] * gnew;
+                r = hs[kHist - tD1 + s] * gnew;
+                if(sameFilter && oldOn && uint32_t(s) < fademix)
+                {
+                    const float gold = oldStep*float(fademix - uint32_t(s));
+                    l += hs[kHist - oD0 + s] * gold;
+                    r += hs[kHist - oD1 + s] * gold;
+                }
+            }
+            S.lLR[i] = make_float2(l, r);
+        }
+        const bool oldPass = !sameFilter && oldOn;
+        if(oldPass)
+            for(int i = t;i < Smem::kOLen;i += GS)
+            {
+                const int s = i - FP;
+                float l = 0.0f, r = 0.0f;
+                if(s >= 0 && uint32_t(s) < fademix)
+                {
+                    const float gold = oldStep*float(fademix - uint32_t(s));
+                    l = hs[kHist - oD0 + s] * gold;
+                    r = hs[kHist - oD1 + s] * gold;
+                }
+                S.oLR[i] = make_float2(l, r);
+            }
+        group_sync(bar, GS);
+
+        {
+            const uint32_t o2 = oi + 2u*stride, o1 = oi + stride;
+            const uint32_t v2 = o2 < P.num_order ? P.order[o2] : 0xffffffffu;
+            const uint32_t v1 = o1 < P.num_order ? P.order[o1] : 0xffffffffu;
+            if(v2 < P.max_voices)
+            {
+                if(t < 5) prefetch_l2(reinterpret_cast<const char*>(&P.voices[v2]) + t*128);
+                else if(t < 5 + int((P.ir_pad*8u + 127u)/128u))
+                    prefetch_l2(reinterpret_cast<const char*>(P.hrtf_tgt + size_t(v2)*P.ir_pad) + (t-5)*128);
+            }
+            if(v1 < P.max_voices && t < int(kLine*sizeof(float)/128u))
+            {
+                const float *nl = ((P.sendinfo[v1] & kSiDeferred) ? P.dline : P.xscratch) + size_t(v1)*kLine;
+                prefetch_l2(reinterpret_cast<const char*>(nl) + t*128);
+            }
+        }
+
+        const int irpad = int(P.ir_pad);
+        fir_pass<OPT, FP>(acc, S.lLR, S.coefT, irpad, t0);
+        if(oldPass && t0 < int(kHist) + irpad)
+            fir_pass<OPT, FP>(acc, S.oLR, S.coefO, irpad, t0);
+        if(t == 0)
+        {
+            rec.old_delay0 = tD0; rec.old_delay1 = tD1;
+            rec.old_gain = targetGain;
+        }
+        group_sync(bar, GS);
+    }
+
+    const size_t row = blockIdx.x;
+    __syncthreads();
+    float *stage = reinterpret_cast<float*>(smem_raw);
+    for(int gg = 0;gg < GROUPS;++gg)
+    {
+        if(g == gg)
+        {
+            #pragma unroll
+            for(int r = 0;r < OPT;++r)
+            {
+                const int o = t0 + r;
+                if(o < kAccumLen)
+                {
+                    if(gg == 0) { stage[o] = acc[r].x; stage[kAccumLen + o] = acc[r].y; }
+                    else { stage[o] += acc[r].x; stage[kAccumLen + o] += acc[r].y; }
+                }
+            }
+            if(gg == 0 && GS*OPT < kAccumLen)
+                for(int o = GS*OPT + t;o < kAccumLen;o += GS) { stage[o] = 0.0f; stage[kAccumLen + o] = 0.0f; }
+        }
+        __syncthreads();
+    }
+    float *pl = P.partial + row*(2*kAccumLen);
+    for(int o = threadIdx.x;o < 2*kAccumLen;o += GS*GROUPS) pl[o] = stage[o];
+}
+
 
 constexpr int kReduceCols = 8, kReduceSegs = 128;
 __global__ void __launch_bounds__(1024)
```
